# rnaarla/advanced-rag-milvus

Measured on AMD Instinct MI355X. Metric: queries_per_sec_hybrid_retrieve, higher is better.
Workload: dtype f16

## Files before the change

advanced-rag-milvus_amd/advanced_rag/_native.py:

```python
from __future__ import annotations

import ctypes
import os
import threading
from typing import Optional, Sequence, Tuple

import numpy as np

from .staging import csr_of_queries

HR_F32, HR_F16 = 0, 1
HR_METRIC_IP, HR_METRIC_COSINE, HR_METRIC_L2 = 0, 1, 2
HR_METHOD_SEMANTIC, HR_METHOD_SPARSE, HR_METHOD_DOMAIN = 1, 2, 4
HR_MAX_TOPK = 256
HR_NORM_COSINE, HR_NORM_ATAN, HR_NORM_ATAN_DIST, HR_NORM_MINMAX, HR_NORM_MINMAX_DIST = 0, 1, 2, 3, 4
HR_MAX_FUSE_LISTS = 16
HR_FUSE_RRF, HR_FUSE_WEIGHTED = 0, 1
HR_DECAY_GAUSS, HR_DECAY_EXP, HR_DECAY_LINEAR = 0, 1, 2
HR_NORM_NONE = -1
HR_MAX_BOOST_FUNCS = 8
HR_BOOST_ACTIVE, HR_BOOST_RANDOM = 1, 2
HR_BOOST_MULTIPLY, HR_BOOST_SUM = 0, 1
HR_COL_F64 = 5
HR_MAX_DEEP_K = 16384
HR_N_PHASES = 10
PHASE_NAMES = ("prep", "dense_scan", "group_select", "refine", "topk",
               "sparse_scan", "sparse_select", "sparse_refine", "sparse_topk", "finish_fused")
HR_DEBUG_FINISH_MODE, HR_DEBUG_FAIL_NEXT_BUILD, HR_DEBUG_DENSE_KERNELS, HR_DEBUG_SPARSE_RPB, HR_DEBUG_GROUP_ROWS = 1, 2, 3, 4, 5
HR_DEBUG_NO_TRIM = 6
HR_DEBUG_NO_RANGE_CLAMP = 7

_HERE = os.path.dirname(os.path.abspath(__file__))
LIB_PATH = os.path.join(os.path.dirname(_HERE), "lib", "libhbmrag.so")

_lib = None
_lib_lock = threading.Lock()


class HbmRagError(RuntimeError):

    def __init__(self, status: int, message: str):
        super().__init__(f"libhbmrag status {status}: {message}")
        self.status = status


_c = ctypes
_SIGNATURES = {
    "hr_version": (_c.c_int, []),
    "hr_create": (_c.c_int, [_c.c_int, _c.c_int64, _c.c_int, _c.c_int, _c.c_int64, _c.POINTER(_c.c_void_p)]),
    "hr_destroy": (None, [_c.c_void_p]),
    "hr_last_error": (_c.c_char_p, [_c.c_void_p]),
    "hr_set_row_offset": (_c.c_int, [_c.c_void_p, _c.c_int64]),
    "hr_reserve": (_c.c_int, [_c.c_void_p, _c.c_int64]),
    "hr_add_dense": (_c.c_int, [_c.c_void_p, _c.c_void_p, _c.c_int64]),
    "hr_add_dense_raw": (_c.c_int, [_c.c_void_p, _c.c_void_p, _c.c_int64]),
    "hr_add_dense_raw_dev": (_c.c_int, [_c.c_void_p, _c.c_void_p, _c.c_int64, _c.c_void_p]),
    "hr_add_sparse": (_c.c_int, [_c.c_void_p, _c.c_void_p, _c.c_void_p, _c.c_void_p, _c.c_int64]),
    "hr_finalize": (_c.c_int, [_c.c_void_p]),
    "hr_compact": (_c.c_int, [_c.c_void_p, _c.c_void_p, _c.c_int, _c.POINTER(_c.c_int64), _c.POINTER(_c.c_int64)]),
    "hr_save": (_c.c_int, [_c.c_void_p, _c.c_char_p]),
    "hr_load": (_c.c_int, [_c.c_char_p, _c.c_int, _c.POINTER(_c.c_void_p)]),
    "hr_get_info": (_c.c_int, [_c.c_void_p, _c.POINTER(_c.c_int64), _c.POINTER(_c.c_int32), _c.POINTER(_c.c_int32),
                               _c.POINTER(_c.c_int64)]),
    "hr_num_rows": (_c.c_int64, [_c.c_void_p]),
    "hr_num_sparse_rows": (_c.c_int64, [_c.c_void_p]),
    "hr_device_bytes": (_c.c_int64, [_c.c_void_p]),
    "hr_dense_scan_bytes": (_c.c_int64, [_c.c_void_p]),
    "hr_search_dense": (_c.c_int, [_c.c_void_p, _c.c_void_p, _c.c_int, _c.c_int, _c.c_void_p, _c.c_void_p,
                                   _c.c_void_p]),
    "hr_search_dense_range": (_c.c_int, [_c.c_void_p, _c.c_void_p, _c.c_int, _c.c_int, _c.c_void_p, _c.c_int, _c.c_void_p,
                                         _c.c_void_p, _c.c_void_p, _c.c_void_p]),
    "hr_search_sparse": (_c.c_int, [_c.c_void_p, _c.c_void_p, _c.c_void_p, _c.c_void_p, _c.c_int, _c.c_int,
                                    _c.c_float, _c.c_void_p, _c.c_void_p, _c.c_void_p]),
    "hr_search_dense_dmask": (_c.c_int, [_c.c_void_p, _c.c_void_p, _c.c_int, _c.c_int, _c.c_void_p, _c.c_void_p,
                                         _c.c_void_p]),
    "hr_search_sparse_dmask": (_c.c_int, [_c.c_void_p, _c.c_void_p, _c.c_void_p, _c.c_void_p, _c.c_int, _c.c_int,
                                          _c.c_float, _c.c_void_p, _c.c_void_p, _c.c_void_p]),
    "hr_filter_eval_expr_dev": (_c.c_int, [_c.c_void_p, _c.c_int, _c.c_void_p, _c.c_int, _c.c_int64, _c.c_void_p, _c.c_void_p,
                                           _c.c_void_p, _c.c_void_p, _c.c_void_p]),
    "hr_filter_eval_dev": (_c.c_int, [_c.c_void_p, _c.c_int, _c.c_int64, _c.c_void_p, _c.c_void_p, _c.c_void_p,
                                      _c.c_void_p, _c.c_void_p]),
    "hr_bm25_encode_dev": (_c.c_int, [_c.c_void_p, _c.c_void_p, _c.c_int, _c.c_int, _c.c_double, _c.c_double, _c.c_double, _c.c_int,
                                      _c.c_void_p, _c.c_void_p, _c.c_void_p, _c.c_void_p, _c.c_void_p]),
    "hr_hash_tokenize_dev": (_c.c_int, [_c.c_void_p, _c.c_void_p, _c.c_int, _c.c_int, _c.c_int, _c.c_void_p, _c.c_void_p, _c.c_void_p,
                                        _c.c_void_p]),
    "hr_fuse_rrf": (_c.c_int, [_c.c_void_p, _c.c_void_p, _c.c_int, _c.c_void_p, _c.c_int, _c.c_void_p, _c.c_int,
                               _c.c_double, _c.c_double, _c.c_double, _c.c_int, _c.c_void_p, _c.c_void_p,
                               _c.c_void_p, _c.c_void_p]),
    "hr_fuse_scores": (_c.c_int, [_c.c_void_p] + [_c.c_void_p, _c.c_void_p, _c.c_int, _c.c_int] * 3 +
                       [_c.c_double, _c.c_double, _c.c_double, _c.c_void_p, _c.c_void_p, _c.c_void_p, _c.c_void_p]),
    "hr_fuse_scores_dev": (_c.c_int, [_c.c_void_p, _c.c_void_p, _c.c_int, _c.c_int] * 3 +
                           [_c.c_int, _c.c_double, _c.c_double, _c.c_double, _c.c_void_p, _c.c_int, _c.c_void_p,
                            _c.c_void_p, _c.c_void_p, _c.c_void_p, _c.c_void_p]),
    "hr_fuse_lists_dev": (_c.c_int, [_c.c_void_p, _c.c_void_p, _c.c_int, _c.c_int, _c.c_int, _c.c_int, _c.c_int, _c.c_void_p,
                                     _c.c_void_p, _c.c_void_p, _c.c_int, _c.c_void_p, _c.c_void_p, _c.c_void_p, _c.c_void_p,
                                     _c.c_void_p]),
    "hr_search_dense_dev": (_c.c_int, [_c.c_void_p, _c.c_void_p, _c.c_int, _c.c_int, _c.c_void_p, _c.c_void_p,
                                       _c.c_void_p, _c.c_void_p, _c.c_void_p]),
    "hr_search_dense_range_dev": (_c.c_int, [_c.c_void_p, _c.c_void_p, _c.c_int, _c.c_int, _c.c_void_p, _c.c_void_p,
                                             _c.c_void_p, _c.c_void_p, _c.c_void_p, _c.c_void_p, _c.c_void_p]),
    "hr_search_sparse_dev": (_c.c_int, [_c.c_void_p, _c.c_void_p, _c.c_void_p, _c.c_void_p, _c.c_int, _c.c_int64,
                                        _c.c_int, _c.c_int, _c.c_void_p, _c.c_void_p, _c.c_void_p, _c.c_void_p,
                                        _c.c_void_p]),
    "hr_search_hybrid_dev": (_c.c_int, [_c.c_void_p, _c.c_void_p, _c.c_void_p, _c.c_void_p, _c.c_void_p, _c.c_int,
                                        _c.c_int64, _c.c_int, _c.c_int, _c.c_void_p, _c.c_void_p, _c.c_void_p,
                                        _c.c_void_p, _c.c_void_p]),
    "hr_hybrid_prep_dev": (_c.c_int, [_c.c_void_p, _c.c_void_p, _c.c_void_p, _c.c_void_p, _c.c_void_p, _c.c_int,
                                      _c.c_int64, _c.c_int, _c.c_int, _c.c_int, _c.c_void_p]),
    "hr_hybrid_scan_dev": (_c.c_int, [_c.c_void_p, _c.c_void_p, _c.c_void_p, _c.c_void_p, _c.c_void_p, _c.c_int,
                                      _c.c_int64, _c.c_int, _c.c_int, _c.c_void_p, _c.c_int, _c.c_void_p]),
    "hr_hybrid_finish_dev": (_c.c_int, [_c.c_void_p, _c.c_void_p, _c.c_void_p, _c.c_void_p, _c.c_void_p, _c.c_int,
                                        _c.c_int, _c.c_int, _c.c_void_p, _c.c_int, _c.c_void_p, _c.c_void_p,
                                        _c.c_void_p, _c.c_void_p]),
    "hr_fuse_rrf_dev": (_c.c_int, [_c.c_void_p, _c.c_int, _c.c_void_p, _c.c_int, _c.c_void_p, _c.c_int, _c.c_int,
                                   _c.c_double, _c.c_double, _c.c_double, _c.c_int, _c.c_int, _c.c_void_p,
                                   _c.c_void_p, _c.c_void_p, _c.c_void_p, _c.c_void_p]),
    "hr_merge_topk_dev": (_c.c_int, [_c.c_void_p, _c.c_void_p, _c.c_int, _c.c_int64, _c.c_int64, _c.c_int, _c.c_int,
                                     _c.c_int, _c.c_void_p, _c.c_void_p, _c.c_void_p]),
    "hr_merge_topk_asc_dev": (_c.c_int, [_c.c_void_p, _c.c_void_p, _c.c_int, _c.c_int64, _c.c_int64, _c.c_int, _c.c_int,
                                     _c.c_int, _c.c_void_p, _c.c_void_p, _c.c_void_p]),
    "hr_post_lists_dev": (_c.c_int, [_c.c_void_p, _c.c_int, _c.c_void_p]),
    "hr_stream_create": (_c.c_int, [_c.c_int, _c.c_int, _c.c_void_p, _c.c_int, _c.POINTER(_c.c_void_p)]),
    "hr_stream_destroy": (_c.c_int, [_c.c_int, _c.c_void_p]),
    "hr_set_scan_cus": (_c.c_int, [_c.c_void_p, _c.c_int]),
    "hr_debug_option": (_c.c_int, [_c.c_void_p, _c.c_int, _c.c_int]),
    "hr_rerank_linear_dev": (_c.c_int, [_c.c_void_p, _c.c_void_p, _c.c_void_p, _c.c_void_p, _c.c_void_p, _c.c_int,
                                        _c.c_int, _c.c_double, _c.c_double, _c.c_double, _c.c_int, _c.c_void_p,
                                        _c.c_void_p, _c.c_void_p, _c.c_void_p]),
    "hr_mmr_select_dev": (_c.c_int, [_c.c_void_p, _c.c_void_p, _c.c_void_p, _c.c_int, _c.c_int, _c.c_void_p, _c.c_void_p,
                                     _c.c_int64, _c.c_int64, _c.c_void_p, _c.c_int, _c.c_void_p, _c.c_void_p, _c.c_void_p]),
    "hr_mmr_vec_scratch_bytes": (_c.c_size_t, [_c.c_void_p, _c.c_int, _c.c_int]),
    "hr_mmr_select_vec_dev": (_c.c_int, [_c.c_void_p, _c.c_void_p, _c.c_void_p, _c.c_int, _c.c_int, _c.c_void_p, _c.c_int, _c.c_int,
                                         _c.c_void_p, _c.c_int, _c.c_void_p, _c.c_void_p, _c.c_void_p, _c.c_void_p, _c.c_void_p]),
    "hr_group_select_dev": (_c.c_int, [_c.c_void_p, _c.c_void_p, _c.c_int, _c.c_int, _c.c_void_p, _c.c_int64, _c.c_int64, _c.c_int,
                                       _c.c_void_p, _c.c_void_p, _c.c_void_p, _c.c_void_p, _c.c_void_p]),
    "hr_boost_rerank_dev": (_c.c_int, [_c.c_void_p, _c.c_void_p, _c.c_int, _c.c_void_p, _c.c_int, _c.c_int, _c.c_void_p, _c.c_int,
                                       _c.c_int64, _c.c_int, _c.c_int, _c.c_int, _c.c_int, _c.c_int, _c.c_void_p, _c.c_void_p,
                                       _c.c_void_p, _c.c_void_p, _c.c_void_p, _c.c_void_p]),
    "hr_decay_rerank_dev": (_c.c_int, [_c.c_void_p, _c.c_void_p, _c.c_int, _c.c_void_p, _c.c_int, _c.c_int, _c.c_void_p, _c.c_int,
                                       _c.c_int64, _c.c_int64, _c.c_void_p, _c.c_int, _c.c_int, _c.c_void_p, _c.c_void_p, _c.c_void_p,
                                       _c.c_void_p, _c.c_void_p]),
    "hr_mask_drop_groups_dev": (_c.c_int, [_c.c_void_p, _c.c_void_p, _c.c_int64, _c.c_void_p, _c.c_void_p, _c.c_int, _c.c_void_p]),
    "hr_group_select_n_dev": (_c.c_int, [_c.c_void_p, _c.c_void_p, _c.c_int, _c.c_int, _c.c_void_p, _c.c_int64, _c.c_int64, _c.c_int,
                                         _c.c_int, _c.c_void_p, _c.c_void_p, _c.c_void_p, _c.c_void_p, _c.c_void_p, _c.c_void_p]),
    "hr_mask_keep_groups_dev": (_c.c_int, [_c.c_void_p, _c.c_void_p, _c.c_int64, _c.c_void_p, _c.c_void_p, _c.c_int, _c.c_void_p]),
    "hr_add_layernorm_f16_dev": (_c.c_int, [_c.c_void_p, _c.c_void_p, _c.c_void_p, _c.c_void_p, _c.c_void_p, _c.c_int64,
                                            _c.c_int, _c.c_float, _c.c_void_p]),
    "hr_embed_layernorm_f16_dev": (_c.c_int, [_c.c_void_p, _c.c_void_p, _c.c_void_p, _c.c_void_p, _c.c_void_p, _c.c_void_p,
                                              _c.c_void_p, _c.c_void_p, _c.c_int64, _c.c_int, _c.c_int, _c.c_float, _c.c_int64,
                                              _c.c_int64, _c.c_void_p]),
    "hr_attention_f16_dev": (_c.c_int, [_c.c_void_p, _c.c_void_p, _c.c_void_p, _c.c_int64, _c.c_int, _c.c_int, _c.c_int,
                                        _c.c_float, _c.c_void_p]),
    "hr_attention_rows_f16_dev": (_c.c_int, [_c.c_void_p, _c.c_int64, _c.c_int64, _c.c_void_p, _c.c_void_p, _c.c_int64, _c.c_int64,
                                             _c.c_void_p, _c.c_void_p, _c.c_int64, _c.c_int, _c.c_int, _c.c_int, _c.c_int, _c.c_float,
                                             _c.c_void_p]),
    "hr_linear_rows_f16_dev": (_c.c_int, [_c.c_void_p, _c.c_int, _c.c_void_p, _c.c_void_p, _c.c_void_p, _c.c_int64, _c.c_int, _c.c_int,
                                          _c.c_int64, _c.c_void_p]),
    "hr_attention_fr_f16_dev": (_c.c_int, [_c.c_void_p, _c.c_void_p, _c.c_void_p, _c.c_int64, _c.c_int, _c.c_int, _c.c_int,
                                           _c.c_float, _c.c_void_p]),
    "hr_encoder_tail_f16_dev": (_c.c_int, [_c.c_void_p, _c.c_void_p, _c.c_int, _c.c_void_p, _c.c_int, _c.c_void_p, _c.c_void_p,
                                           _c.c_int64, _c.c_int, _c.c_int, _c.c_float, _c.c_int, _c.c_void_p]),
    "hr_mask_rows_scratch_bytes": (_c.c_size_t, [_c.c_int64]),
    "hr_mask_rows_dev": (_c.c_int, [_c.c_void_p, _c.c_int64, _c.c_int64, _c.c_int64, _c.c_int64, _c.c_void_p, _c.c_void_p,
                                    _c.c_void_p, _c.c_void_p]),
    "hr_get_dense_rows_dev": (_c.c_int, [_c.c_void_p, _c.c_void_p, _c.c_int64, _c.c_int, _c.c_void_p, _c.c_int64, _c.c_void_p,
                                         _c.c_void_p]),
    "hr_get_dense_rows": (_c.c_int, [_c.c_void_p, _c.c_void_p, _c.c_int64, _c.c_void_p]),
    "hr_get_sparse_rows_scratch_bytes": (_c.c_size_t, [_c.c_int64]),
    "hr_get_sparse_rows_dev": (_c.c_int, [_c.c_void_p, _c.c_void_p, _c.c_int64, _c.c_void_p, _c.c_void_p, _c.c_void_p, _c.c_int64,
                                          _c.c_void_p, _c.c_void_p, _c.c_void_p]),
    "hr_get_sparse_rows": (_c.c_int, [_c.c_void_p, _c.c_void_p, _c.c_int64, _c.c_void_p, _c.c_void_p, _c.c_void_p, _c.c_int64,
                                      _c.c_void_p]),
    "hr_search_dense_deep": (_c.c_int, [_c.c_void_p, _c.c_void_p, _c.c_int, _c.c_int, _c.c_int, _c.c_void_p, _c.c_int, _c.c_void_p,
                                        _c.c_void_p]),
    "hr_search_sparse_deep": (_c.c_int, [_c.c_void_p, _c.c_void_p, _c.c_void_p, _c.c_void_p, _c.c_int, _c.c_int, _c.c_int,
                                         _c.c_float, _c.c_void_p, _c.c_int, _c.c_void_p, _c.c_void_p]),
    "hr_deep_topk_scratch_bytes": (_c.c_size_t, [_c.c_int64, _c.c_int, _c.c_int]),
    "hr_deep_topk_dev": (_c.c_int, [_c.c_void_p, _c.c_void_p, _c.c_int64, _c.c_int, _c.c_int, _c.c_int, _c.c_int, _c.c_int64,
                                    _c.c_void_p, _c.c_void_p, _c.c_void_p, _c.c_void_p]),
    "hr_search_dense_deep_after": (_c.c_int, [_c.c_void_p, _c.c_void_p, _c.c_int, _c.c_int, _c.c_void_p, _c.c_void_p, _c.c_void_p,
                                              _c.c_void_p, _c.c_void_p, _c.c_void_p, _c.c_int, _c.c_void_p, _c.c_void_p]),
    "hr_search_sparse_deep_after": (_c.c_int, [_c.c_void_p, _c.c_void_p, _c.c_void_p, _c.c_void_p, _c.c_int, _c.c_int, _c.c_void_p,
                                               _c.c_void_p, _c.c_void_p, _c.c_float, _c.c_void_p, _c.c_int, _c.c_void_p,
                                               _c.c_void_p]),
    "hr_deep_topk_window_dev": (_c.c_int, [_c.c_void_p, _c.c_void_p, _c.c_int64, _c.c_int, _c.c_int, _c.c_int, _c.c_int64,
                                           _c.c_void_p, _c.c_void_p, _c.c_void_p, _c.c_void_p, _c.c_void_p]),
    "hr_set_profiling": (_c.c_int, [_c.c_void_p, _c.c_int]),
    "hr_last_kernel_ms": (_c.c_int, [_c.c_void_p, _c.c_void_p, _c.c_int]),
    "hr_last_compact_ms": (_c.c_int, [_c.c_void_p, _c.c_void_p, _c.c_int]),
}
EXPORTED_SYMBOLS = tuple(_SIGNATURES)


def load_library(path: Optional[str] = None) -> ctypes.CDLL:
    global _lib
    with _lib_lock:
        if _lib is not None and path is None:
            return _lib
        p = path or os.environ.get("HBMRAG_LIB", LIB_PATH)
        if not os.path.exists(p):
            raise FileNotFoundError(
                f"{p} not found: build it with `make -C advanced-rag-milvus_amd` "
                "(or __graft_entry__.build()); there is no CPU fallback")
        try:
            import torch
        except Exception:
            pass
        L = ctypes.CDLL(p)
        for name, (restype, argtypes) in _SIGNATURES.items():
            fn = getattr(L, name)
            fn.restype = restype
            fn.argtypes = argtypes
        if path is None:
            _lib = L
        return L


def _vp(a) -> Optional[ctypes.c_void_p]:
    if a is None:
        return None
    if isinstance(a, np.ndarray):
        return a.ctypes.data_as(ctypes.c_void_p)
    return ctypes.c_void_p(int(a))


class ShardHandle:

    def __init__(self, dim: int, dtype: int = HR_F16, metric: int = HR_METRIC_COSINE, sparse_dim: int = 0,
                 device: int = 0, _adopt: Optional[int] = None):
        self._lib = load_library()
        self._h = ctypes.c_void_p()
        if _adopt is not None:
            self._h = ctypes.c_void_p(_adopt)
            self.dim, self.dtype, self.metric, self.sparse_dim, self.device = dim, dtype, metric, sparse_dim, device
            return
        self.dim, self.dtype, self.metric, self.sparse_dim, self.device = dim, dtype, metric, sparse_dim, device
        rc = self._lib.hr_create(device, dim, dtype, metric, sparse_dim, ctypes.byref(self._h))
        if rc != 0:
            msg = (self._lib.hr_last_error(None) or b"").decode()
            self._h = ctypes.c_void_p()
            self._raise(rc, msg)

    def _raise(self, rc: int, msg: Optional[str] = None):
        if msg is None:
            msg = (self._lib.hr_last_error(self._h) or b"").decode()
        if rc == 1:
            raise ValueError(msg)
        raise HbmRagError(rc, msg)

    def _check(self, rc: int):
        if rc != 0:
            self._raise(rc)

    def close(self):
        if getattr(self, "_h", None) is not None and self._h.value:
            self._lib.hr_destroy(self._h)
            self._h = ctypes.c_void_p()

    def __del__(self):
        try:
            self.close()
        except Exception:
            pass

    def save(self, path: str):
        self._check(self._lib.hr_save(self._h, os.fsencode(path)))

    @classmethod
    def load(cls, path: str, dim: int, dtype: int = HR_F16, metric: int = HR_METRIC_COSINE, sparse_dim: int = 0,
             device: int = 0) -> "ShardHandle":
        lib = load_library()
        h = ctypes.c_void_p()
# ... 260 lines not shown
        os_ = np.empty(cap, dtype=np.float64)
        om = np.empty(cap, dtype=np.int32)
        n = ctypes.c_int32(0)
        self._check(self._lib.hr_fuse_rrf(self._h, _vp(a) if len(a) else None, len(a), _vp(b) if len(b) else None,
                                          len(b), _vp(c) if len(c) else None, len(c), wa, wb, wc, rrf_k, _vp(oi),
                                          _vp(os_), _vp(om), ctypes.byref(n)))
        return oi[:n.value].copy(), os_[:n.value].copy(), om[:n.value].copy()

    def fuse_scores(self, lists, norms, weights=(0.7, 0.3, 0.2)):
        lists = list(lists) + [((), ())] * (3 - len(lists))
        norms = list(norms) + [HR_NORM_COSINE] * (3 - len(norms))
        w = list(weights) + [0.0] * (3 - len(weights))
        ids = [np.ascontiguousarray(l[0], dtype=np.int64) for l in lists]
        sc = [np.ascontiguousarray(l[1], dtype=np.float32) for l in lists]
        if any(len(i) != len(s) for i, s in zip(ids, sc)):
            raise ValueError("a list's ids and scores differ in length")
        cap = max(sum(len(i) for i in ids), 1)
        oi = np.empty(cap, dtype=np.int64)
        os_ = np.empty(cap, dtype=np.float64)
        om = np.empty(cap, dtype=np.int32)
        n = ctypes.c_int32(0)
        args = []
        for i, s, code in zip(ids, sc, norms):
            args += [_vp(i) if len(i) else None, _vp(s) if len(i) else None, len(i), int(code)]
        self._check(self._lib.hr_fuse_scores(self._h, *args, float(w[0]), float(w[1]), float(w[2]), _vp(oi), _vp(os_),
                                             _vp(om), ctypes.byref(n)))
        return oi[:n.value].copy(), os_[:n.value].copy(), om[:n.value].copy()

    def search_dense_dev(self, d_q: int, B: int, k: int, d_ids: int, d_scores: int, d_flags: int = 0,
                         d_rowmask: int = 0, stream: int = 0):
        self._check(self._lib.hr_search_dense_dev(self._h, _vp(d_q), B, k, _vp(d_rowmask) if d_rowmask else None,
                                                  _vp(d_ids), _vp(d_scores), _vp(d_flags) if d_flags else None,
                                                  _vp(stream) if stream else None))

    def search_dense_range_dev(self, d_q: int, B: int, k: int, d_radius: int, d_range_filter: int, d_ids: int,
                               d_scores: int, d_flags: int = 0, d_rowmask: int = 0, stream: int = 0):
        self._check(self._lib.hr_search_dense_range_dev(
            self._h, _vp(d_q), B, k, _vp(d_rowmask) if d_rowmask else None, _vp(d_radius) if d_radius else None,
            _vp(d_range_filter) if d_range_filter else None, _vp(d_ids), _vp(d_scores),
            _vp(d_flags) if d_flags else None, _vp(stream) if stream else None))

    def search_sparse_dev(self, d_indptr: int, d_idx: int, d_val: int, B: int, nnz_total: int, max_q_nnz: int, k: int,
                          d_ids: int, d_scores: int, d_flags: int = 0, d_rowmask: int = 0, stream: int = 0):
        self._check(self._lib.hr_search_sparse_dev(self._h, _vp(d_indptr), _vp(d_idx), _vp(d_val), B, nnz_total,
                                                   max_q_nnz, k, _vp(d_rowmask) if d_rowmask else None, _vp(d_ids),
                                                   _vp(d_scores), _vp(d_flags) if d_flags else None,
                                                   _vp(stream) if stream else None))

    def search_hybrid_dev(self, d_q: int, d_indptr: int, d_idx: int, d_val: int, B: int, nnz_total: int,
                          max_q_nnz: int, k: int, d_ids: int, d_scores: int, d_flags: int = 0, d_rowmask: int = 0,
                          stream: int = 0):
        self._check(self._lib.hr_search_hybrid_dev(self._h, _vp(d_q), _vp(d_indptr), _vp(d_idx) if d_idx else None,
                                                   _vp(d_val) if d_val else None, B, nnz_total, max_q_nnz, k,
                                                   _vp(d_rowmask) if d_rowmask else None, _vp(d_ids), _vp(d_scores),
                                                   _vp(d_flags) if d_flags else None, _vp(stream) if stream else None))

    def hybrid_prep_dev(self, d_q: int, d_indptr: int, d_idx: int, d_val: int, B: int, nnz_total: int, max_q_nnz: int,
                        k: int, slot: int, stream: int = 0):
        self._check(self._lib.hr_hybrid_prep_dev(self._h, _vp(d_q), _vp(d_indptr), _vp(d_idx) if d_idx else None,
                                                 _vp(d_val) if d_val else None, B, nnz_total, max_q_nnz, k, slot,
                                                 _vp(stream) if stream else None))

    def hybrid_scan_dev(self, d_q: int, d_indptr: int, d_idx: int, d_val: int, B: int, nnz_total: int, max_q_nnz: int,
                        k: int, slot: int, stream: int = 0, d_rowmask: int = 0):
        self._check(self._lib.hr_hybrid_scan_dev(self._h, _vp(d_q), _vp(d_indptr), _vp(d_idx) if d_idx else None,
                                                 _vp(d_val) if d_val else None, B, nnz_total, max_q_nnz, k,
                                                 _vp(d_rowmask) if d_rowmask else None, slot,
                                                 _vp(stream) if stream else None))

    def hybrid_finish_dev(self, d_q: int, d_indptr: int, d_idx: int, d_val: int, B: int, max_q_nnz: int, k: int,
                          slot: int, d_ids: int, d_scores: int, d_flags: int = 0, stream: int = 0, d_rowmask: int = 0):
        self._check(self._lib.hr_hybrid_finish_dev(self._h, _vp(d_q), _vp(d_indptr), _vp(d_idx) if d_idx else None,
                                                   _vp(d_val) if d_val else None, B, max_q_nnz, k,
                                                   _vp(d_rowmask) if d_rowmask else None, slot, _vp(d_ids),
                                                   _vp(d_scores), _vp(d_flags) if d_flags else None,
                                                   _vp(stream) if stream else None))

    def set_scan_cus(self, n_cus: int):
        self._check(self._lib.hr_set_scan_cus(self._h, int(n_cus)))

    def debug_option(self, key: int, value: int):
        self._check(self._lib.hr_debug_option(self._h, key, value))

    def set_profiling(self, level: int):
        self._check(self._lib.hr_set_profiling(self._h, level))

    def kernel_ms(self):
        buf = np.zeros(2 * HR_N_PHASES, dtype=np.float32)
        self._check(self._lib.hr_last_kernel_ms(self._h, _vp(buf), buf.shape[0]))
        return {PHASE_NAMES[p]: (float(buf[p]), int(buf[HR_N_PHASES + p])) for p in range(HR_N_PHASES)}

    def compact_ms(self):
        buf = np.zeros(3, dtype=np.float32)
        self._check(self._lib.hr_last_compact_ms(self._h, _vp(buf), 3))
        return {"tile_gather": float(buf[0]), "call": float(buf[1]), "posting_rebuild": float(buf[2])}


def fuse_rrf_dev(d_a: int, ka: int, d_b: int, kb: int, d_c: int, kc: int, B: int, wa: float, wb: float, wc: float,
                 rrf_k: int, top_k: int, d_out_ids: int, d_out_scores: int, d_out_methods: int, d_n_out: int,
                 stream: int = 0):
    L = load_library()
    rc = L.hr_fuse_rrf_dev(_vp(d_a) if ka else None, ka, _vp(d_b) if kb else None, kb, _vp(d_c) if kc else None, kc,
                           B, wa, wb, wc, rrf_k, top_k, _vp(d_out_ids), _vp(d_out_scores), _vp(d_out_methods),
                           _vp(d_n_out), _vp(stream) if stream else None)
    if rc != 0:
        msg = (L.hr_last_error(None) or b"").decode()
        if rc == 1:
            raise ValueError(msg)
        raise HbmRagError(rc, msg)


def _raise_global(L, rc: int):
    msg = (L.hr_last_error(None) or b"").decode()
    if rc == 1:
        raise ValueError(msg)
    raise HbmRagError(rc, msg)


def fuse_scores_dev(d_a: int, d_sa: int, ka: int, norm_a: int, d_b: int, d_sb: int, kb: int, norm_b: int, d_c: int,
                    d_sc: int, kc: int, norm_c: int, B: int, wa: float, wb: float, wc: float, d_w_query: int, top_k: int,
                    d_out_ids: int, d_out_scores: int, d_out_methods: int, d_n_out: int, stream: int = 0):
    L = load_library()
    p = lambda v: _vp(v) if v else None
    rc = L.hr_fuse_scores_dev(p(d_a), p(d_sa), ka, norm_a, p(d_b), p(d_sb), kb, norm_b, p(d_c), p(d_sc), kc, norm_c, B,
                              wa, wb, wc, p(d_w_query), top_k, p(d_out_ids), p(d_out_scores), p(d_out_methods),
                              p(d_n_out), p(stream))
    if rc != 0:
        _raise_global(L, rc)


def fuse_lists_dev(d_ids: int, d_scores: int, n_lists: int, k_in: int, B: int, mode: int, rrf_k: int, norms, weights,
                   d_w_query: int, top_k: int, d_out_ids: int, d_out_scores: int, d_out_lists: int, d_n_out: int,
                   stream: int = 0):
    L = load_library()
    p = lambda v: _vp(v) if v else None
    h_norms = None if norms is None else np.ascontiguousarray(norms, dtype=np.int32)
    h_w = None if weights is None else np.ascontiguousarray(weights, dtype=np.float64)
    for name, arr in (("norms", h_norms), ("weights", h_w)):
        if arr is not None and arr.shape != (max(int(n_lists), 0),):
            raise ValueError(f"{name} must hold one value per list ({n_lists}), got shape {arr.shape}")
    rc = L.hr_fuse_lists_dev(p(d_ids), p(d_scores), n_lists, k_in, B, mode, rrf_k, _vp(h_norms), _vp(h_w), p(d_w_query),
                             top_k, p(d_out_ids), p(d_out_scores), p(d_out_lists), p(d_n_out), p(stream))
    if rc != 0:
        _raise_global(L, rc)


def mmr_select_dev(d_ids: int, d_scores: int, d_n: int, B: int, k_in: int, d_tok_indptr: int, d_tok: int, tok_rows: int,
                   first_row: int, d_lambda: int, k_out: int, d_out_pos: int, d_out_n: int, stream: int = 0):
    L = load_library()
    rc = L.hr_mmr_select_dev(_vp(d_ids) if d_ids else None, _vp(d_scores) if d_scores else None, _vp(d_n) if d_n else None,
                             B, k_in, _vp(d_tok_indptr) if d_tok_indptr else None, _vp(d_tok) if d_tok else None,
                             tok_rows, first_row, _vp(d_lambda) if d_lambda else None, k_out,
                             _vp(d_out_pos) if d_out_pos else None, _vp(d_out_n) if d_out_n else None,
                             _vp(stream) if stream else None)
    if rc != 0:
        _raise_global(L, rc)


def group_select_dev(d_ids: int, d_n: int, B: int, k_in: int, d_keys: int, key_rows: int, first_row: int, k_out: int,
                     d_out_pos: int, d_out_keys: int, d_out_n: int, d_flags: int, stream: int = 0):
    L = load_library()
    p = lambda x: _vp(x) if x else None
    rc = L.hr_group_select_dev(p(d_ids), p(d_n), B, k_in, p(d_keys), key_rows, first_row, k_out, p(d_out_pos), p(d_out_keys),
                               p(d_out_n), p(d_flags), p(stream))
    if rc != 0:
        _raise_global(L, rc)
# ... 308 lines not shown
```

advanced-rag-milvus_amd/csrc/finish.h:

```cpp
#pragma once
#include "common.h"
#include "dense.h"
#include "select.h"
#include "sparse.h"

namespace hbmrag {

constexpr int kFinishThreads = 512;
constexpr int kFinishMaxSlots = 4096;
constexpr int kFinishMaxCand = 256;
constexpr int kFinishMaxBuckets = 12288;

struct FinishMod {
    int kind;
    int group_rows;
    GroupSelArgs sel;
    TopkArgs topk;
    const uint8_t* rowmask;
    const chunk_t* tiles;
    int KT, dim, metric, dtype;
    const float* q;
    const double* qn2;
    const double* norm2;
    const double* range_bounds;
    const int64_t* indptr;
    const int32_t* idx;
    const float* val;
    const int64_t* q_indptr;
    const int32_t* q_idx;
    const float* q_val;
    int q_cap;
    int64_t n_rows;
};
struct FinishPair {
    FinishMod m[2];
    int n;
    int key_slots;
};

__host__ __device__ inline bool finish_sparse_hashed(int q_cap) { return q_cap <= kHashMaxTerms; }
inline size_t finish_lds_bytes(const FinishPair& p) {
    size_t region_b = 0;
    for (int i = 0; i < p.n; ++i) {
        const FinishMod& m = p.m[i];
        if (m.sel.two_level) region_b = region_b > (size_t)m.sel.n_buckets * 4 ? region_b : (size_t)m.sel.n_buckets * 4;
        if (m.kind == 1) {
            const size_t s = (size_t)kFilterBits / 8 +
                             (finish_sparse_hashed(m.q_cap) ? (size_t)sparse_hash_slots(m.q_cap) * 8 : (size_t)m.q_cap * 8);
            region_b = region_b > s ? region_b : s;
        } else {
            const size_t s = (size_t)m.dim * 4;
            region_b = region_b > s ? region_b : s;
        }
    }
    return (size_t)p.key_slots * 8 + region_b;
}

constexpr int kFinishBucketsPerWave = 32;
__device__ inline void bucket_max_block(const GroupSelArgs& a, int q, float* s_bmax) {
    const int lane = threadIdx.x & 63;
    const int wid = __builtin_amdgcn_readfirstlane((int)(threadIdx.x >> 6)), nw = blockDim.x >> 6;
    const float* gm = a.gmax + (int64_t)q * a.n_groups;
    for (int64_t b0 = (int64_t)wid * kFinishBucketsPerWave; b0 < a.n_buckets; b0 += (int64_t)nw * kFinishBucketsPerWave) {
        float v[kFinishBucketsPerWave];
#pragma unroll
        for (int i = 0; i < kFinishBucketsPerWave; ++i) {
            const int64_t g = (b0 + i) * kBucketGroups + lane;
            v[i] = g < a.n_groups ? gm[g] : -__builtin_inff();
        }
        float mine = -__builtin_inff();
#pragma unroll
        for (int i = 0; i < kFinishBucketsPerWave; ++i) {
            const float m = wave_max_dpp(v[i]);
            if (lane == i) mine = m;
        }
        if (lane < kFinishBucketsPerWave && b0 + lane < a.n_buckets) s_bmax[b0 + lane] = mine;
    }
}

#ifdef HR_STAMP
__device__ unsigned long long hr_finish_stamps[2][8];
#define FINISH_STAMP(i)                                                                      \
    do {                                                                                     \
        if (blockIdx.x == 0 && threadIdx.x == 0) hr_finish_stamps[blockIdx.y][i] = __builtin_amdgcn_s_memtime(); \
    } while (0)
#else
#define FINISH_STAMP(i) do {} while (0)
#endif

__global__ __launch_bounds__(kFinishThreads) void finish_kernel(FinishPair p) {
    extern __shared__ uint64_t finish_lds[];
    __shared__ SelectScratch sh;
    __shared__ int32_t sel_bucket[HR_MAX_TOPK * 2];
    __shared__ uint64_t sel[HR_MAX_TOPK];
    __shared__ int32_t s_cand[kFinishMaxCand];
    const FinishMod& a = p.m[blockIdx.y];
    const int q = blockIdx.x, tid = threadIdx.x;
    const int n_slots = a.sel.C * a.group_rows;
    uint64_t* s_key = finish_lds;
    float* s_bmax = reinterpret_cast<float*>(finish_lds + p.key_slots);

    FINISH_STAMP(0);
    if (a.sel.two_level) bucket_max_block(a.sel, q, s_bmax);
    __syncthreads();
    FINISH_STAMP(1);
    select_groups_block(a.sel, q, s_bmax, s_cand, sh, sel_bucket);
    __syncthreads();
    const int n_live_slots = min(sh.n_live, a.sel.C) * a.group_rows;
    for (int slot = n_live_slots + tid; slot < n_slots; slot += kFinishThreads) s_key[slot] = 0ull;
    FINISH_STAMP(2);
#ifdef HR_STAMP
    if (blockIdx.x == 0 && tid == 0) {
        hr_finish_stamps[blockIdx.y][5] = (unsigned long long)n_live_slots;
        hr_finish_stamps[blockIdx.y][6] = 0ull;
    }
#endif

    if (a.kind == 0) {
        float* qq = s_bmax;
        for (int k = tid; k < a.dim; k += kFinishThreads) qq[k] = a.q[(int64_t)q * a.dim + k];
        __syncthreads();
        const double qn2 = a.qn2[q];
        const double* rq = a.range_bounds ? a.range_bounds + 2 * q : nullptr;
        for (int slot = tid; slot < n_live_slots; slot += kFinishThreads) {
#ifdef HR_STAMP
            if (blockIdx.x == 0) atomicAdd(&hr_finish_stamps[blockIdx.y][6], 1ull);
#endif
            float sc = 0.f;
            int32_t row = -1;
            bool ok;
            if (a.metric == HR_METRIC_L2)
                ok = a.dtype == HR_F16
                         ? refine_dense_slot<_Float16, true>(a.tiles, a.KT, a.dim, qq, qn2, a.norm2, a.rowmask, s_cand,
                                                             a.group_rows, a.n_rows, a.metric, slot, &sc, &row)
                         : refine_dense_slot<float, true>(a.tiles, a.KT, a.dim, qq, qn2, a.norm2, a.rowmask, s_cand,
                                                          a.group_rows, a.n_rows, a.metric, slot, &sc, &row);
            else
                ok = a.dtype == HR_F16
                         ? refine_dense_slot<_Float16>(a.tiles, a.KT, a.dim, qq, qn2, a.norm2, a.rowmask, s_cand,
                                                       a.group_rows, a.n_rows, a.metric, slot, &sc, &row)
                         : refine_dense_slot<float>(a.tiles, a.KT, a.dim, qq, qn2, a.norm2, a.rowmask, s_cand,
                                                    a.group_rows, a.n_rows, a.metric, slot, &sc, &row);
            if (ok && rq) ok = a.metric == HR_METRIC_L2 ? dense_score_in_range<true>(sc, rq) : dense_score_in_range<false>(sc, rq);
            s_key[slot] = ok ? rank_key(sc, (uint32_t)row) : 0ull;
        }
    } else {
        constexpr int NW = kFinishThreads / 64;
        const int n_chains = NW * ((n_live_slots + NW * 64 - 1) / (NW * 64));
        const int chain_len = (n_live_slots + n_chains - 1) / n_chains;
        const int wid = __builtin_amdgcn_readfirstlane(tid >> 6);
        auto emit = [&](int slot, bool keep, float score, int64_t doc) { s_key[slot] = keep ? rank_key(score, (uint32_t)doc) : 0ull; };
        if (finish_sparse_hashed(a.q_cap)) {
            const int hs = sparse_hash_slots(a.q_cap);
            unsigned int* s_filter = reinterpret_cast<unsigned int*>(s_bmax);
            int32_t* s_hkey = reinterpret_cast<int32_t*>(s_filter + kFilterBits / 32);
            float* s_hval = reinterpret_cast<float*>(s_hkey + hs);
            refine_sparse_stage_query_hash(a.q_indptr, a.q_idx, a.q_val, q, a.q_cap, hs, s_filter, s_hkey, s_hval);
            for (int chain = wid; chain < n_chains; chain += NW) {
                const int slot0 = chain * chain_len;
                const int n_here = min(chain_len, n_live_slots - slot0);
                if (n_here > 0)
                    refine_sparse_chain(a.indptr, a.idx, a.val, a.rowmask, s_cand, a.group_rows, a.n_rows, slot0, n_here,
                                        SparseLookupHash{s_filter, s_hkey, s_hval, hs}, emit);
            }
        } else {
            unsigned int* s_filter = reinterpret_cast<unsigned int*>(s_bmax);
            int32_t* s_idx = reinterpret_cast<int32_t*>(s_filter + kFilterBits / 32);
            float* s_val = reinterpret_cast<float*>(s_idx + a.q_cap);
            const int nt = refine_sparse_stage_query(a.q_indptr, a.q_idx, a.q_val, q, a.q_cap, s_filter, s_idx, s_val);
            for (int chain = wid; chain < n_chains; chain += NW) {
                const int slot0 = chain * chain_len;
                const int n_here = min(chain_len, n_live_slots - slot0);
                if (n_here > 0)
                    refine_sparse_chain(a.indptr, a.idx, a.val, a.rowmask, s_cand, a.group_rows, a.n_rows, slot0, n_here,
                                        SparseLookupSorted{s_filter, s_idx, s_val, nt}, emit);
            }
        }
    }
    __syncthreads();
    FINISH_STAMP(3);
    TopkArgs t = a.topk;
    t.n = n_slots;
    select_topk_block(t, q, [&](int64_t i) -> uint64_t { return s_key[i]; }, sh, sel);
    __syncthreads();
    FINISH_STAMP(4);
}

}
```

advanced-rag-milvus_amd/csrc/hbmrag.hip:

```cpp
#include "../../include/hbmrag.h"

#include <hip/hip_runtime.h>

#include <algorithm>
#include <chrono>
#include <cmath>
#include <cstdarg>
#include <cstdio>
#include <cstdlib>
#include <cstring>
#include <map>
#include <mutex>
#include <new>
#include <shared_mutex>
#include <string>
#include <type_traits>
#include <utility>
#include <vector>

#include "common.h"
#include "attention.h"
#include "boost.h"
#include "compact.h"
#include "decay.h"
#include "deep.h"
#include "encoder_layer.h"
#include "scan_plan.h"
#include "dense.h"
#include "encoder_ops.h"
#include "filter.h"
#include "finish.h"
#include "fuse.h"
#include "fuse_lists.h"
#include "group.h"
#include "mmr.h"
#include "query.h"
#include "text.h"
#include "select.h"
#include "sparse.h"

using namespace hbmrag;

namespace {

thread_local std::string g_last_error;

struct DevBuf {
    void* p = nullptr;
    size_t cap = 0;
    DevBuf() = default;
    DevBuf(const DevBuf&) = delete;
    DevBuf& operator=(const DevBuf&) = delete;
    DevBuf(DevBuf&& o) noexcept : p(o.p), cap(o.cap) { o.p = nullptr, o.cap = 0; }
    DevBuf& operator=(DevBuf&& o) noexcept {
        if (this != &o) {
            release();
            p = o.p, cap = o.cap;
            o.p = nullptr, o.cap = 0;
        }
        return *this;
    }
    ~DevBuf() { release(); }
    hipError_t alloc_exact(size_t bytes) {
        release();
        hipError_t e = hipMalloc(&p, bytes);
        if (e == hipSuccess) cap = bytes;
        else p = nullptr;
        return e;
    }
    hipError_t ensure(size_t bytes) { return bytes <= cap ? hipSuccess : alloc_exact(bytes + bytes / 8 + 256); }
    hipError_t grow(size_t bytes, size_t keep, hipStream_t s) {
        if (bytes <= cap) return hipSuccess;
        DevBuf nb;
        hipError_t e = nb.alloc_exact(bytes + bytes / 2 + 256);
        if (e == hipSuccess && p && keep) {
            e = hipMemcpyAsync(nb.p, p, keep, hipMemcpyDeviceToDevice, s);
            if (e == hipSuccess) e = hipStreamSynchronize(s);
        }
        if (e == hipSuccess) *this = std::move(nb);
        return e;
    }
    void release() {
        if (p) (void)hipFree(p);
        p = nullptr;
        cap = 0;
    }
    template <typename T> T* as() const { return reinterpret_cast<T*>(p); }
};

enum Phase { PH_PREP = 0, PH_SCAN, PH_GSEL, PH_REFINE, PH_TOPK, PH_SSCAN, PH_SGSEL, PH_SREFINE, PH_STOPK, PH_FINISH, PH_COUNT };
static_assert(PH_COUNT == HR_N_PHASES, "phase table and ABI out of step");

struct WorkspaceQueues {
    hipStream_t stream = nullptr;
    hipStream_t side = nullptr;
    hipEvent_t ev_scan = nullptr, ev_side = nullptr;
    ~WorkspaceQueues() {
        if (stream) (void)hipStreamDestroy(stream);
        if (side) (void)hipStreamDestroy(side);
        if (ev_scan) (void)hipEventDestroy(ev_scan);
        if (ev_side) (void)hipEventDestroy(ev_side);
    }
};

struct Workspace : WorkspaceQueues {
    std::mutex mu;
    int users = 0;
    struct Workspace* sparse_ws = nullptr;
    DevBuf qfrag, qn2, gmax, bmax, cand, acut, cscore, crow, flags, qscale, qeps, qfloor, pq_n, pq_idx, pq_w;
    DevBuf qcoef, dqeps;
    DevBuf rbounds, rhi, rlo;
    DevBuf d_radius, d_rfilter;
    DevBuf d_q, d_ids, d_scores, d_mask;
    DevBuf d_qptr, d_qidx, d_qval;
    DevBuf f_ids, f_sc, f_out_ids, f_out_scores, f_out_meth, f_n;
    ~Workspace() { delete sparse_ws; }
};

struct EventSpan {
    int phase;
    hipEvent_t a, b;
};

}

struct hr_index {
    int device = 0;
    int64_t dim = 0, sparse_dim = 0;
    int dtype = HR_F16, metric = HR_METRIC_COSINE;
    int KT = 0;
    int group_rows_override = 0;
    int64_t row_offset = 0;

    DevBuf tiles, scale, norm2, max_norm;
    int64_t cap_rows = 0, n_rows = 0, n_normed = 0;
    float max_row_norm = 0.f;
    DevBuf stage;
    DevBuf bad_row;
    hipStream_t ingest_stream = nullptr;

    std::vector<int64_t> pend_indptr{0};
    std::vector<int32_t> pend_idx;
    std::vector<float> pend_val;
    std::vector<int64_t> h_range_base{0};
    std::vector<unsigned> h_range_dense;
    int64_t n_sparse = 0, n_csr = 0, nnz_csr = 0, n_sparse_built = 0;
    float max_sparse_abs = 0.f;
    bool sparse_signed = false;
    DevBuf s_indptr, s_idx, s_val, rt_off, range_base, post;
    DevBuf idle_post;
    int64_t n_ranges = 0;
    int64_t n_dense_runs = 0;

    bool finalized = false;
    int profiling = 0;
    int cu_count = 256;
    int scan_cus = 0;
    int fault_inject = 0;
    float compact_ms[3] = {};
    bool slot_prepped[HR_MAX_SLOTS] = {};

    mutable std::shared_mutex rw;
    std::mutex pool_mu;
    std::vector<Workspace*> free_ws;
    std::map<void*, Workspace*> stream_ws;
    Workspace* slot_ws[HR_MAX_SLOTS][2] = {};
    std::mutex prof_mu;
    std::vector<EventSpan> spans;
    std::vector<hipEvent_t> event_pool;
    mutable std::mutex err_mu;
    mutable std::string err;

    ~hr_index() {
        for (Workspace* w : free_ws) delete w;
        for (auto& kv : stream_ws) delete kv.second;
        for (auto& pair : slot_ws)
            for (Workspace* w : pair) delete w;
        for (auto& sp : spans) { (void)hipEventDestroy(sp.a); (void)hipEventDestroy(sp.b); }
        for (hipEvent_t e : event_pool) (void)hipEventDestroy(e);
        if (ingest_stream) (void)hipStreamDestroy(ingest_stream);
    }
};

namespace {

int fail(const hr_index* h, int code, const char* fmt, ...) {
    char buf[512];
    va_list ap;
    va_start(ap, fmt);
    vsnprintf(buf, sizeof buf, fmt, ap);
    va_end(ap);
    if (h) {
        std::lock_guard<std::mutex> g(h->err_mu);
        h->err = buf;
    }
    g_last_error = buf;
    return code;
}

#define HIP_TRY(h, expr)                                                                   \
    do {                                                                                   \
        hipError_t e__ = (expr);                                                           \
        if (e__ != hipSuccess) return fail(h, HR_EHIP, "%s: %s", #expr, hipGetErrorString(e__)); \
    } while (0)

#define HR_TRY(expr)               \
    do {                           \
        int rc__ = (expr);         \
        if (rc__ != HR_OK) return rc__; \
    } while (0)

inline size_t elem_size(int dtype) { return dtype == HR_F16 ? 2 : 4; }
inline int elems_per_chunk(int dtype) { return dtype == HR_F16 ? 8 : 4; }
inline int64_t round_up(int64_t x, int64_t m) { return (x + m - 1) / m * m; }
inline size_t tile_bytes_for_rows(const hr_index* h, int64_t rows) {
    return (size_t)(rows / kRowsPerBlock) * h->KT * 1024;
}

struct DeviceGuard {
// ... 161 lines not shown
}

template <int KT, int NRB, int GW, int NW>
hipError_t launch_scan_qreg(const ScanArgs& a) {
    const hr_index* h = a.h;
    const int64_t blocks = std::max<int64_t>(1, std::min<int64_t>(a.n_super, (int64_t)scan_cus(h) * (8 / NW)));
    hipLaunchKernelGGL((dense_scan_qreg_kernel<KT, NRB, GW, NW>), dim3((unsigned)blocks), dim3(64 * NW), 0, a.s,
                       h->tiles.as<chunk_t>(), a.qfrag, h->scale.as<float>(), a.mask, a.gmax, a.nq, h->n_rows, a.n_super);
    return hipGetLastError();
}
template <int NRB>
hipError_t launch_scan_q64(const ScanArgs& a) {
    const hr_index* h = a.h;
    const int64_t blocks = std::max<int64_t>(1, std::min<int64_t>(a.n_super, (int64_t)scan_cus(h)));
    const size_t lds = (size_t)kQregStages * 24 * 1024 + 2 * kSuperRows * sizeof(float);
    static bool ready = false;
    if (!ready) {
        hipError_t e = hipFuncSetAttribute((const void*)dense_scan_q64_kernel<24, NRB>, hipFuncAttributeMaxDynamicSharedMemorySize, (int)lds);
        if (e != hipSuccess) return e;
        ready = true;
    }
    hipLaunchKernelGGL((dense_scan_q64_kernel<24, NRB>), dim3((unsigned)blocks), dim3(256), lds, a.s, h->tiles.as<chunk_t>(),
                       a.qfrag, h->scale.as<float>(), a.mask, a.gmax, a.nq, h->n_rows, a.n_super);
    return hipGetLastError();
}
template <int NRB>
hipError_t launch_scan_gemm(const ScanArgs& a) {
    const hr_index* h = a.h;
    const int64_t n_tiles = (a.n_super * kRowBlocksPerSuper + kGemmRowBlocks - 1) / kGemmRowBlocks;
    const unsigned blocks = (unsigned)std::max<int64_t>(1, std::min<int64_t>(n_tiles, scan_cus(h)));
    hipLaunchKernelGGL((dense_scan_gemm_kernel<16, NRB>), dim3(blocks), dim3(512), 0, a.s, h->tiles.as<chunk_t>(), a.qfrag,
                       h->scale.as<float>(), a.mask, a.gmax, a.nq, h->KT, h->n_rows, a.n_super);
    return hipGetLastError();
}

template <int... Vs, typename F>
hipError_t with_constant(int v, F f) {
    hipError_t e = hipErrorInvalidValue;
    (void)((v == Vs ? (e = f(std::integral_constant<int, Vs>{}), true) : false) || ...);
    return e;
}

template <typename F>
auto with_store(int dtype, F f) {
    if (dtype == HR_F16) return f(_Float16{});
    return f(float{});
}

template <typename STORE, bool L2, bool RANGE>
hipError_t launch_scan_generic(const ScanPlan& p, const ScanArgs& a) {
    return with_constant<1, 4>(p.NRB, [&](auto nrb) {
        if (p.kind == SCAN_BIGQ) return launch_scan_bigq<STORE, 8, decltype(nrb)::value, L2, RANGE>(a);
        return with_constant<1, 2, 3, 4>(
            p.G, [&](auto g) { return launch_scan_lds<STORE, decltype(g)::value, decltype(nrb)::value, L2, RANGE>(a); });
    });
}

hipError_t launch_scan(const ScanPlan& p, const ScanArgs& a) {
    switch (p.kind) {
        case SCAN_QREG: return with_constant<1, 4>(p.NRB, [&](auto nrb) { return launch_scan_qreg<24, decltype(nrb)::value, 2, 8>(a); });
        case SCAN_Q64: return with_constant<1, 4>(p.NRB, [&](auto nrb) { return launch_scan_q64<decltype(nrb)::value>(a); });
        case SCAN_GEMM: return with_constant<1, 4>(p.NRB, [&](auto nrb) { return launch_scan_gemm<decltype(nrb)::value>(a); });
        case SCAN_LDS:
        case SCAN_BIGQ:
            return with_store(a.h->dtype, [&](auto store) {
                using STORE = decltype(store);
                if (p.range) return p.l2 ? launch_scan_generic<STORE, true, true>(p, a) : launch_scan_generic<STORE, false, true>(p, a);
                return p.l2 ? launch_scan_generic<STORE, true, false>(p, a) : launch_scan_generic<STORE, false, false>(p, a);
            });
        default: return hipErrorInvalidValue;
    }
}

struct DenseRange {
    const double* d_radius;
    const double* d_range_filter;
};

int g_dense_kernels = 0;
int g_sparse_rpb = 0;
int g_no_trim = 0;
int g_group_rows = 0;
int g_no_range_clamp = 0;

inline int64_t bucket_count(int64_t n_groups) { return (n_groups + kBucketGroups - 1) / kBucketGroups; }
int launch_group_select_pair(hr_index* h, hipStream_t s, int B, const GroupSelPair& p) {
    int64_t blocks = 0;
    for (int m = 0; m < p.n; ++m)
        if (p.m[m].two_level) blocks = std::max(blocks, (p.m[m].n_buckets + 4 * kBucketsPerWave - 1) / (4 * kBucketsPerWave));
    if (blocks > 0) {
        hipLaunchKernelGGL(bucket_max_kernel, dim3((unsigned)blocks, B, p.n), dim3(256), 0, s, p);
        HIP_TRY(h, hipGetLastError());
    }
    hipLaunchKernelGGL(select_groups_kernel, dim3(B, p.n), dim3(1024), 0, s, p);
    HIP_TRY(h, hipGetLastError());
    return HR_OK;
}
int launch_topk_pair(hr_index* h, hipStream_t s, int B, const TopkPair& p) {
    hipLaunchKernelGGL(select_topk_kernel, dim3(B, p.n), dim3(1024), 0, s, p);
    HIP_TRY(h, hipGetLastError());
    return HR_OK;
}

constexpr int kMaxSelectGroups = 448;
int next_candidate_count(int C, int64_t n_groups) {
    const int64_t all = round_up(n_groups, 16);
    if (C < kMaxSelectGroups && (int64_t)C * 4 < all) return std::min(C * 4, kMaxSelectGroups);
    return (int)all;
}

int candidate_groups_for_k(int k) {
    int c = k + std::max(16, k / 2);
    return (int)round_up(c, 16);
}

float dense_l2_rt_eps(const hr_index* h) {
    const double M = (double)h->max_row_norm * 1.0001;
    return (float)std::min(std::ldexp(1.0, -22) * 1.01 * 0.5 * M * M, 3.0e38);
}
void dense_eps(const hr_index* h, float* eps_abs, int* norm_mode) {
    const double Dp = (double)h->KT * 4 * elems_per_chunk(h->dtype);
    double unit = 2.0 * Dp * std::ldexp(1.0, -24) + 1e-6;
    unit += (h->dtype == HR_F16) ? std::ldexp(1.0, -11) * 1.01
                                 : std::ldexp(1.0, -22);
    if (h->metric == HR_METRIC_COSINE) {
        *eps_abs = (float)unit;
        *norm_mode = 0;
    } else if (h->metric == HR_METRIC_L2) {
        *eps_abs = (float)((unit + std::ldexp(1.0, -24) * 1.01) * (double)h->max_row_norm * 1.0001);
        *norm_mode = 2;
    } else {
        *eps_abs = (float)(unit * (double)h->max_row_norm * 1.0001);
        *norm_mode = 1;
    }
}

struct OutLists {
    int64_t* ids;
    float* scores;
    int32_t* flags;
};
struct FinishSide {
    Workspace* ws;
    bool sparse;
    int GR;
    int64_t n_groups;
    int C;
    const uint8_t* mask;
    TopkArgs topk;
    const float* d_q;
    const double* range_bounds;
    const int64_t* q_ptr;
    const int32_t* q_idx;
    const float* q_val;
    int stride;
    int ph_select, ph_refine, ph_topk;
};

int side_common(hr_index* h, Workspace* ws, int B, int k, int C, int GR, int64_t n_groups, const uint8_t* d_mask,
                const OutLists& out, FinishSide* f) {
    HIP_TRY(h, ws->gmax.ensure((size_t)B * n_groups * sizeof(float)));
    HIP_TRY(h, ws->bmax.ensure((size_t)B * bucket_count(n_groups) * sizeof(float)));
    HIP_TRY(h, ws->cand.ensure((size_t)B * C * sizeof(int32_t)));
    HIP_TRY(h, ws->acut.ensure((size_t)B * sizeof(float)));
    HIP_TRY(h, ws->cscore.ensure((size_t)B * C * GR * sizeof(float)));
    HIP_TRY(h, ws->crow.ensure((size_t)B * C * GR * sizeof(int32_t)));
    *f = FinishSide{};
    f->ws = ws;
    f->GR = GR;
    f->n_groups = n_groups;
    f->C = C;
    f->mask = d_mask;
    TopkArgs& t = f->topk;
    t.cscore = ws->cscore.as<float>();
    t.crow = ws->crow.as<int32_t>();
    t.n = C * GR;
    t.K = k;
    t.row_offset = h->row_offset;
    t.a_cut = ws->acut.as<float>();
    t.out_ids = out.ids;
    t.out_scores = out.scores;
    t.flags = out.flags;
    return HR_OK;
}
inline int64_t dense_super_groups(const hr_index* h) { return (h->n_rows + kSuperRows - 1) / kSuperRows; }
int dense_side(hr_index* h, Workspace* ws, const float* d_q, int B, int k, int C, const uint8_t* d_mask, const OutLists& out,
               FinishSide* f, bool ranged = false) {
    const int GR = group_rows_for(h, h->n_rows);
    HR_TRY(side_common(h, ws, B, k, C, GR, dense_super_groups(h) * (kSuperRows / GR), d_mask, out, f));
    f->d_q = d_q;
    f->ph_select = PH_GSEL, f->ph_refine = PH_REFINE, f->ph_topk = PH_TOPK;
    TopkArgs& t = f->topk;
    dense_eps(h, &t.eps_abs, &t.norm_mode);
    t.cut_floor = -INFINITY;
    t.eps_abs_q = t.norm_mode == 2 ? ws->dqeps.as<float>() : nullptr;
    t.qn2 = ws->qn2.as<double>();
    if (ranged) {
        f->range_bounds = ws->rbounds.as<double>();
        t.cut_floor_q = ws->rlo.as<float>();
    }
    return HR_OK;
}
int sparse_side(hr_index* h, Workspace* ws, const int64_t* d_qptr, const int32_t* d_qidx, const float* d_qval, int B,
                int max_q_nnz, int k, int C, const uint8_t* d_mask, const OutLists& out, FinishSide* f) {
    const int GR = group_rows_for(h, h->n_sparse);
    HR_TRY(side_common(h, ws, B, k, C, GR, (h->n_sparse + GR - 1) / GR, d_mask, out, f));
    f->sparse = true;
    f->q_ptr = d_qptr;
    f->q_idx = d_qidx;
    f->q_val = d_qval;
    f->stride = (int)round_up(std::max(max_q_nnz, 1), 64);
    f->ph_select = PH_SGSEL, f->ph_refine = PH_SREFINE, f->ph_topk = PH_STOPK;
    TopkArgs& t = f->topk;
    t.cut_floor_q = ws->qfloor.as<float>();
    t.eps_abs_q = ws->qeps.as<float>();
    t.eps_rel = (float)(std::ldexp(1.0, -11) * 1.01 + std::ldexp(1.0, -22));
    return HR_OK;
}

GroupSelArgs sel_args(const FinishSide& f) {
    GroupSelArgs a{};
    a.gmax = f.ws->gmax.as<float>();
    a.bmax = f.ws->bmax.as<float>();
    a.n_groups = f.n_groups;
    a.n_buckets = bucket_count(f.n_groups);
    a.C = f.C;
    a.two_level = f.n_groups > f.C && a.n_buckets > f.C;
    a.cand = f.ws->cand.as<int32_t>();
    a.a_cut = f.ws->acut.as<float>();
    a.K_trim = g_no_trim ? 0 : f.topk.K;
    a.eps_abs = f.topk.eps_abs;
    a.eps_rel = f.topk.eps_rel;
    a.eps_abs_q = f.topk.eps_abs_q;
    return a;
}
FinishMod finish_mod(const hr_index* h, const FinishSide& f) {
    FinishMod m{};
    m.kind = f.sparse;
    m.group_rows = f.GR;
    m.sel = sel_args(f);
    m.topk = f.topk;
    m.rowmask = f.mask;
    if (f.sparse) {
        m.indptr = h->s_indptr.as<int64_t>();
        m.idx = h->s_idx.as<int32_t>();
        m.val = h->s_val.as<float>();
        m.q_indptr = f.q_ptr;
        m.q_idx = f.q_idx;
        m.q_val = f.q_val;
        m.q_cap = f.stride;
        m.n_rows = h->n_sparse;
    } else {
        m.tiles = h->tiles.as<chunk_t>();
        m.KT = h->KT;
        m.dim = (int)h->dim;
        m.metric = h->metric;
        m.dtype = h->dtype;
        m.q = f.d_q;
        m.qn2 = f.ws->qn2.as<double>();
        m.norm2 = h->norm2.as<double>();
        m.range_bounds = f.range_bounds;
        m.n_rows = h->n_rows;
    }
    return m;
}
struct RefineBufs {
    const double* qn2;
    const int32_t* cand;
    float* cscore;
    int32_t* crow;
};
int launch_refine(hr_index* h, hipStream_t s, int B, const FinishSide& f, const RefineBufs& b) {
    if (!f.sparse) {
        const bool f16 = h->dtype == HR_F16, l2 = h->metric == HR_METRIC_L2;
        auto kern = f16 ? (l2 ? refine_dense_kernel<_Float16, true> : refine_dense_kernel<_Float16, false>)
                        : (l2 ? refine_dense_kernel<float, true> : refine_dense_kernel<float, false>);
        hipLaunchKernelGGL(kern, dim3((f.C * f.GR + 63) / 64, B), dim3(64), 0, s, h->tiles.as<chunk_t>(), h->KT, (int)h->dim,
                           f.d_q, b.qn2, h->norm2.as<double>(), f.mask, b.cand, f.C, f.GR,
                           h->n_rows, h->metric, b.cscore, b.crow, f.range_bounds);
    } else {
        const int dpw = 64;
        const bool hashed = f.stride <= kHashMaxTerms;
        const size_t lds = (size_t)kFilterBits / 8 + (hashed ? (size_t)sparse_hash_slots(f.stride) * 8 : (size_t)f.stride * 8);
        hipLaunchKernelGGL(hashed ? refine_sparse_kernel<true> : refine_sparse_kernel<false>,
                           dim3((f.C * f.GR + 4 * dpw - 1) / (4 * dpw), B), dim3(256), lds, s, h->s_indptr.as<int64_t>(),
                           h->s_idx.as<int32_t>(), h->s_val.as<float>(), f.q_ptr, f.q_idx, f.q_val, f.mask,
                           b.cand, f.C, f.GR, h->n_sparse, f.stride, dpw, b.cscore, b.crow);
    }
    HIP_TRY(h, hipGetLastError());
    return HR_OK;
}
int launch_refine(hr_index* h, hipStream_t s, int B, const FinishSide& f) {
    Workspace* ws = f.ws;
    return launch_refine(h, s, B, f, {ws->qn2.as<double>(), ws->cand.as<int32_t>(), ws->cscore.as<float>(), ws->crow.as<int32_t>()});
}

enum { PHASE_SCAN = 1, PHASE_FINISH = 2, PHASE_PREP = 4, PHASE_ALL = 7 };

int g_finish_mode = 0;
bool finish_fused_ok(int B, int n_mod, const FinishSide& f) {
    if (g_finish_mode == 1) return false;
    return ((int64_t)B * n_mod >= 64 || g_finish_mode == 2) && f.C <= kFinishMaxCand && (int64_t)f.C * f.GR <= kFinishMaxSlots &&
           bucket_count(f.n_groups) <= kFinishMaxBuckets;
}
int launch_finish(hr_index* h, hipStream_t s, int B, FinishPair& p) {
    p.key_slots = 0;
    for (int i = 0; i < p.n; ++i) p.key_slots = std::max(p.key_slots, p.m[i].sel.C * p.m[i].group_rows);
    const size_t lds = finish_lds_bytes(p);
    static bool attr_set = false;
    if (!attr_set) {
        HIP_TRY(h, hipFuncSetAttribute((const void*)finish_kernel, hipFuncAttributeMaxDynamicSharedMemorySize, 96 * 1024));
        attr_set = true;
    }
    hipLaunchKernelGGL(finish_kernel, dim3(B, p.n), dim3(kFinishThreads), lds, s, p);
    HIP_TRY(h, hipGetLastError());
    return HR_OK;
}

int finish_enqueue(hr_index* h, hipStream_t s, int B, const FinishSide* f, int n) {
    bool fused = true;
    for (int i = 0; i < n; ++i) fused = fused && finish_fused_ok(B, n, f[i]);
    if (fused) {
        Span sp(h, s, PH_FINISH);
        FinishPair p{};
        p.n = n;
        for (int i = 0; i < n; ++i) p.m[i] = finish_mod(h, f[i]);
        return launch_finish(h, s, B, p);
    }
    {
        Span sp(h, s, f[0].ph_select);
        GroupSelPair p{};
        p.n = n;
        for (int i = 0; i < n; ++i) p.m[i] = sel_args(f[i]);
        HR_TRY(launch_group_select_pair(h, s, B, p));
    }
    for (int i = 0; i < n; ++i) {
        Span sp(h, s, f[i].ph_refine);
        HR_TRY(launch_refine(h, s, B, f[i]));
    }
    {
        Span sp(h, s, f[0].ph_topk);
        TopkPair p{};
        p.n = n;
        for (int i = 0; i < n; ++i) p.m[i] = f[i].topk;
        HR_TRY(launch_topk_pair(h, s, B, p));
    }
    return HR_OK;
}

int dense_search_enqueue(hr_index* h, Workspace* ws, hipStream_t s, const float* d_q, int B, int k,
                         const uint8_t* d_mask, const OutLists& out, int C, hipEvent_t scan_done = nullptr,
                         int phases = PHASE_ALL, const DenseRange* rng = nullptr) {
    const bool ranged = rng != nullptr;
    auto plan_for = [&](int nq) {
        return scan_plan(h->KT, h->dtype, h->metric, h->n_rows, h->group_rows_override, g_dense_kernels, B, nq, ranged);
    };
    const ScanPlan first = plan_for(B);
    if (first.kind == SCAN_NONE)
        return fail(h, HR_ELIMIT, "dim=%lld: the query tile does not fit LDS and the k-chunked pass is switched off",
                    (long long)h->dim);
    const bool l2 = first.l2;
    const int chunk_q = first.chunk_q, Gmax = chunk_q / 16;
    const int n_chunks = (B + chunk_q - 1) / chunk_q;
    const size_t chunk_frag = (size_t)Gmax * h->KT * kTileChunks;
    HIP_TRY(h, ws->qfrag.ensure((size_t)n_chunks * chunk_frag * sizeof(chunk_t)));
    HIP_TRY(h, ws->qn2.ensure((size_t)B * sizeof(double)));
    if (l2) {
        HIP_TRY(h, ws->qcoef.ensure((size_t)n_chunks * chunk_q * sizeof(float)));
        HIP_TRY(h, ws->dqeps.ensure((size_t)n_chunks * chunk_q * sizeof(float)));
    }
    float* const d_coef = l2 ? ws->qcoef.as<float>() : nullptr;
    float* const d_qeps = l2 ? ws->dqeps.as<float>() : nullptr;
    const float rt_eps = l2 ? dense_l2_rt_eps(h) : 0.f;
    RangePrep rp{};
    if (ranged) {
        HIP_TRY(h, ws->rbounds.ensure((size_t)B * 2 * sizeof(double)));
        HIP_TRY(h, ws->rhi.ensure((size_t)n_chunks * chunk_q * sizeof(float)));
        HIP_TRY(h, ws->rlo.ensure((size_t)n_chunks * chunk_q * sizeof(float)));
        int norm_mode;
        dense_eps(h, &rp.eps_abs, &norm_mode);
        rp.radius = rng->d_radius;
        rp.range_filter = rng->d_range_filter;
        rp.bounds = ws->rbounds.as<double>();
        rp.hi_a = ws->rhi.as<float>();
        rp.lo_a = ws->rlo.as<float>();
        rp.max_norm = h->max_row_norm;
        rp.metric = h->metric;
        rp.no_clamp = g_no_range_clamp;
    }
    FinishSide f;
    HR_TRY(dense_side(h, ws, d_q, B, k, C, d_mask, out, &f, ranged));

    if (phases & PHASE_PREP) {
        Span sp(h, s, PH_PREP);
        const int G_total = (n_chunks - 1) * Gmax + plan_for(B - (n_chunks - 1) * chunk_q).G;
        hipLaunchKernelGGL(h->dtype == HR_F16 ? prep_queries_kernel<_Float16> : prep_queries_kernel<float>, dim3(16 * G_total),
                           dim3(256), 0, s, d_q, B, (int)h->dim, h->KT, ws->qfrag.as<chunk_t>(), ws->qn2.as<double>(), d_coef,
                           d_qeps, rt_eps, rp);
        HIP_TRY(h, hipGetLastError());
    }
    for (int c0 = 0; (phases & PHASE_SCAN) && c0 < B; c0 += chunk_q) {
        const int nq = std::min(chunk_q, B - c0);
        Span sp(h, s, PH_SCAN);
        const ScanArgs a{h, s, ws->qfrag.as<chunk_t>() + (size_t)(c0 / chunk_q) * chunk_frag, d_mask,
                         ws->gmax.as<float>() + (int64_t)c0 * f.n_groups, nq, dense_super_groups(h), l2 ? d_coef + c0 : nullptr,
                         ranged ? ws->rhi.as<float>() + c0 : nullptr};
        HIP_TRY(h, launch_scan(plan_for(nq), a));
    }
    if (scan_done) HIP_TRY(h, hipEventRecord(scan_done, s));
    return (phases & PHASE_FINISH) ? finish_enqueue(h, s, B, &f, 1) : HR_OK;
}

int sparse_ranges_per_block(const hr_index* h, int B) {
    const int forced = g_sparse_rpb;
    const int64_t pairs = (int64_t)B * h->n_ranges;
    int64_t rpb = forced > 0 ? forced : std::min<int64_t>(16, pairs / (6 * 2 * (int64_t)scan_cus(h)));
    rpb = std::max<int64_t>(rpb, (h->n_ranges + 65534) / 65535);
    return (int)std::max<int64_t>(1, rpb);
}

int sparse_search_enqueue(hr_index* h, Workspace* ws, hipStream_t s, const int64_t* d_qptr, const int32_t* d_qidx,
                          const float* d_qval, int B, int max_q_nnz, int k, const uint8_t* d_mask, const OutLists& out,
                          int C, int phases = PHASE_ALL) {
    HIP_TRY(h, ws->qscale.ensure((size_t)B * sizeof(float)));
    HIP_TRY(h, ws->qeps.ensure((size_t)B * sizeof(float)));
    HIP_TRY(h, ws->qfloor.ensure((size_t)B * sizeof(float)));
    FinishSide f;
    HR_TRY(sparse_side(h, ws, d_qptr, d_qidx, d_qval, B, max_q_nnz, k, C, d_mask, out, &f));
    if (phases & PHASE_PREP) {
        HIP_TRY(h, ws->pq_n.ensure((size_t)B * 4));
        HIP_TRY(h, ws->pq_idx.ensure((size_t)B * f.stride * 4));
        HIP_TRY(h, ws->pq_w.ensure((size_t)B * f.stride * 4));
        const float max_post_w = h->max_sparse_abs > 0.f ? std::max(h->max_sparse_abs, 0x1p-24f) : 0.f;
        hipLaunchKernelGGL(sparse_query_prep_kernel, dim3(B), dim3(256), 0, s, d_qptr, d_qidx, d_qval, max_post_w,
                           (int)h->sparse_signed, f.stride, (int)h->sparse_dim, ws->qscale.as<float>(),
                           ws->qeps.as<float>(), ws->qfloor.as<float>(), ws->pq_n.as<int32_t>(),
                           ws->pq_idx.as<int32_t>(), ws->pq_w.as<float>());
        HIP_TRY(h, hipGetLastError());
    }
    if (phases & PHASE_SCAN) {
        Span sp(h, s, PH_SSCAN);
        const int rpb = sparse_ranges_per_block(h, B);
        const unsigned chunks = (unsigned)((h->n_ranges + rpb - 1) / rpb);
        hipLaunchKernelGGL(h->n_dense_runs > 0 ? sparse_scan_kernel<true> : sparse_scan_kernel<false>,
                           dim3((unsigned)B, chunks), dim3(kScanThreads), 0, s, h->rt_off.as<unsigned int>(),
                           h->sparse_dim + 1, h->range_base.as<int64_t>(), h->post.as<uint32_t>(), ws->pq_n.as<int32_t>(),
                           ws->pq_idx.as<int32_t>(), ws->pq_w.as<float>(), f.stride, ws->qscale.as<float>(), d_mask,
                           h->n_sparse, f.n_groups, f.GR, h->n_ranges, rpb, h->idle_post.as<uint32_t>(),
                           ws->gmax.as<float>());
        HIP_TRY(h, hipGetLastError());
    }
    return (phases & PHASE_FINISH) ? finish_enqueue(h, s, B, &f, 1) : HR_OK;
}

int check_search_args(hr_index* h, int B, int k, bool dense) {
    if (!h) return fail(nullptr, HR_EINVAL, "null handle");
    if (B <= 0) return fail(h, HR_EINVAL, "batch size must be positive (got %d)", B);
    if (k <= 0) return fail(h, HR_EINVAL, "k must be positive (got %d)", k);
    if (k > HR_MAX_TOPK) return fail(h, HR_ELIMIT, "k=%d exceeds HR_MAX_TOPK=%d", k, HR_MAX_TOPK);
    if (!h->finalized) return fail(h, HR_ESTATE, "search before hr_finalize");
    if (dense && h->dim == 0) return fail(h, HR_ESTATE, "handle has no dense collection");
    if (!dense && h->sparse_dim == 0) return fail(h, HR_ESTATE, "handle has no sparse collection");
    return HR_OK;
}

int fill_empty(hr_index* h, hipStream_t s, int B, int k, int64_t* d_ids, float* d_scores, int32_t* d_flags) {
    HIP_TRY(h, hipMemsetAsync(d_ids, 0xFF, (size_t)B * k * sizeof(int64_t), s));
    HIP_TRY(h, hipMemsetAsync(d_scores, 0, (size_t)B * k * sizeof(float), s));
    if (d_flags) {
        std::vector<int32_t> ones(B, 1);
        HIP_TRY(h, hipMemcpyAsync(d_flags, ones.data(), (size_t)B * sizeof(int32_t), hipMemcpyHostToDevice, s));
        HIP_TRY(h, hipStreamSynchronize(s));
    }
    return HR_OK;
}

struct PooledWs {
    hr_index* h;
    Workspace* w;
    explicit PooledWs(hr_index* h_) : h(h_), w(take_ws(h_)) {}
    ~PooledWs() {
        if (w) give_ws(h, w);
    }
};

template <typename Stage, typename Enqueue>
int search_host(hr_index* h, int B, int k, int64_t hr_index::*rows, const uint8_t* rowmask, bool mask_on_device,
                int64_t* out_ids, float* out_scores, Stage stage_queries, Enqueue enqueue) {
    std::shared_lock<std::shared_mutex> lk(h->rw);
    DeviceGuard dg(h->device);
    const int64_t n_rows = h->*rows;
    if (n_rows == 0) {
        std::fill(out_ids, out_ids + (size_t)B * k, (int64_t)-1);
        std::fill(out_scores, out_scores + (size_t)B * k, 0.f);
        return HR_OK;
    }
    PooledWs pooled(h);
    Workspace* ws = pooled.w;
    if (!ws) return fail(h, HR_ENOMEM, "workspace allocation failed");
    hipStream_t s = ws->stream;
    HR_TRY(stage_queries(ws, s));
    HIP_TRY(h, ws->d_ids.ensure((size_t)B * k * 8));
    HIP_TRY(h, ws->d_scores.ensure((size_t)B * k * 4));
    HIP_TRY(h, ws->flags.ensure((size_t)B * 4));
    const uint8_t* d_mask = mask_on_device ? rowmask : nullptr;
    if (rowmask && !mask_on_device) {
        const size_t mb = (size_t)(n_rows + 7) / 8;
        HIP_TRY(h, ws->d_mask.ensure(mb));
        HIP_TRY(h, hipMemcpyAsync(ws->d_mask.p, rowmask, mb, hipMemcpyHostToDevice, s));
        d_mask = ws->d_mask.as<uint8_t>();
    }
    const OutLists out{ws->d_ids.as<int64_t>(), ws->d_scores.as<float>(), ws->flags.as<int32_t>()};
    const int GR = group_rows_for(h, n_rows);
    const int64_t n_row_groups = (n_rows + GR - 1) / GR;
    int C = candidate_groups_for_k(k);
    std::vector<int32_t> flags(B);
    for (;;) {
        HR_TRY(enqueue(ws, s, d_mask, out, C));
        HIP_TRY(h, hipMemcpyAsync(flags.data(), ws->flags.p, (size_t)B * 4, hipMemcpyDeviceToHost, s));
        HIP_TRY(h, hipStreamSynchronize(s));
        const bool all_exact = std::all_of(flags.begin(), flags.end(), [](int32_t f) { return f != 0; });
        if (all_exact || C >= n_row_groups) break;
        C = next_candidate_count(C, n_row_groups);
    }
    HIP_TRY(h, hipMemcpyAsync(out_ids, out.ids, (size_t)B * k * 8, hipMemcpyDeviceToHost, s));
    HIP_TRY(h, hipMemcpyAsync(out_scores, out.scores, (size_t)B * k * 4, hipMemcpyDeviceToHost, s));
    HIP_TRY(h, hipStreamSynchronize(s));
    return HR_OK;
}

int64_t dense_capacity_for(int64_t cap_rows, int64_t need_rows, bool reserving) {
    const int64_t need = round_up(need_rows, kSuperRows);
    if (reserving && cap_rows == 0) return std::max<int64_t>(need, kSuperRows);
    return std::max<int64_t>({need, round_up(cap_rows + cap_rows / 2, kSuperRows), 1024});
}

int set_dense_capacity(hr_index* h, int64_t rows) {
    DevBuf tiles, scale, norm2;
    const size_t tb = tile_bytes_for_rows(h, rows);
    if (tiles.alloc_exact(tb) != hipSuccess || scale.alloc_exact((size_t)rows * 4) != hipSuccess ||
        norm2.alloc_exact((size_t)rows * 8) != hipSuccess) {
        (void)hipGetLastError();
        return fail(h, HR_ENOMEM, "cannot allocate dense shard for %lld rows (%zu bytes)", (long long)rows, tb);
    }
    hipStream_t s = h->ingest_stream;
    HIP_TRY(h, hipMemsetAsync(tiles.p, 0, tiles.cap, s));
    HIP_TRY(h, hipMemsetAsync(scale.p, 0, scale.cap, s));
    HIP_TRY(h, hipMemsetAsync(norm2.p, 0, norm2.cap, s));
    if (h->cap_rows > 0) {
        HIP_TRY(h, hipMemcpyAsync(tiles.p, h->tiles.p, tile_bytes_for_rows(h, h->cap_rows), hipMemcpyDeviceToDevice, s));
        HIP_TRY(h, hipMemcpyAsync(scale.p, h->scale.p, (size_t)h->cap_rows * 4, hipMemcpyDeviceToDevice, s));
        HIP_TRY(h, hipMemcpyAsync(norm2.p, h->norm2.p, (size_t)h->cap_rows * 8, hipMemcpyDeviceToDevice, s));
    }
    HIP_TRY(h, hipStreamSynchronize(s));
    h->tiles = std::move(tiles);
    h->scale = std::move(scale);
    h->norm2 = std::move(norm2);
    h->cap_rows = rows;
    return HR_OK;
}

int grow_dense(hr_index* h, int64_t need_rows) {
    if (need_rows <= h->cap_rows) return HR_OK;
    return set_dense_capacity(h, dense_capacity_for(h->cap_rows, need_rows, false));
}

constexpr unsigned long long kNoBadRow = ~0ull;

template <typename SRC>
int add_dense_impl(hr_index* h, const SRC* rows, int64_t n, bool src_on_device, hipStream_t user_stream) {
    if (!h) return fail(nullptr, HR_EINVAL, "null handle");
    if (h->dim == 0) return fail(h, HR_ESTATE, "handle has no dense collection");
    if (n < 0 || (n > 0 && !rows)) return fail(h, HR_EINVAL, "bad rows/n");
    if (n == 0) return HR_OK;
    std::unique_lock<std::shared_mutex> lk(h->rw);
    DeviceGuard dg(h->device);
    HR_TRY(grow_dense(h, h->n_rows + n));
    hipStream_t s = src_on_device && user_stream ? user_stream : h->ingest_stream;
    const int64_t chunk_rows = std::max<int64_t>(1, (64ll << 20) / (h->dim * (int64_t)sizeof(SRC)));
    const int kchunks = h->KT * 4;
    unsigned long long* d_bad = h->bad_row.as<unsigned long long>();
    for (int64_t r0 = 0; r0 < n; r0 += chunk_rows) {
        const int64_t m = std::min(chunk_rows, n - r0);
        const SRC* src = rows + r0 * h->dim;
        if (!src_on_device) {
            HIP_TRY(h, h->stage.ensure((size_t)m * h->dim * sizeof(SRC)));
            HIP_TRY(h, hipMemcpyAsync(h->stage.p, src, (size_t)m * h->dim * sizeof(SRC), hipMemcpyHostToDevice, s));
            src = h->stage.as<SRC>();
        }
        const int64_t threads = m * kchunks;
        const unsigned blocks = (unsigned)((threads + 255) / 256);
        with_store(h->dtype, [&](auto store) {
            using STORE = decltype(store);
            using IN = std::conditional_t<std::is_same<STORE, float>::value, float, SRC>;
            hipLaunchKernelGGL((tile_rows_kernel<STORE, IN>), dim3(blocks), dim3(256), 0, s, reinterpret_cast<const IN*>(src), m,
                               (int)h->dim, h->KT, h->n_rows + r0, h->tiles.as<chunk_t>(), r0, d_bad);
        });
        HIP_TRY(h, hipGetLastError());
        if (!src_on_device) HIP_TRY(h, hipStreamSynchronize(s));
    }
    unsigned long long bad = kNoBadRow;
    HIP_TRY(h, hipMemcpyAsync(&bad, d_bad, sizeof bad, hipMemcpyDeviceToHost, s));
    HIP_TRY(h, hipStreamSynchronize(s));
    if (bad != kNoBadRow) {
        const int64_t threads = n * kchunks;
        hipLaunchKernelGGL(zero_rows_kernel, dim3((unsigned)((threads + 255) / 256)), dim3(256), 0, s, n, h->KT,
                           h->n_rows, h->tiles.as<chunk_t>());
        HIP_TRY(h, hipGetLastError());
        HIP_TRY(h, hipMemsetAsync(d_bad, 0xFF, sizeof bad, s));
        HIP_TRY(h, hipStreamSynchronize(s));
        return fail(h, HR_EINVAL, "dense row %lld of the batch holds a value that is NaN or infinite in the shard's %s store",
                    (long long)bad, h->dtype == HR_F16 ? "fp16" : "fp32");
    }
    h->n_rows += n;
    h->finalized = false;
    return HR_OK;
}

int validate_csr(const hr_index* h, const int64_t* indptr, const int32_t* indices, const float* values, int64_t n,
                 float* batch_max, bool* batch_neg) {
    float mx = 0.f;
    bool neg = false;
    for (int64_t r = 0; r < n; ++r) {
        if (indptr[r + 1] < indptr[r]) return fail(h, HR_EINVAL, "indptr not monotone at row %lld", (long long)r);
        int32_t prev = -1;
        for (int64_t e = indptr[r]; e < indptr[r + 1]; ++e) {
            const int32_t t = indices[e];
            if (t < 0 || t >= h->sparse_dim)
                return fail(h, HR_EINVAL, "sparse index %d out of range [0,%lld) in row %lld", t, (long long)h->sparse_dim, (long long)r);
            if (t <= prev) return fail(h, HR_EINVAL, "sparse indices must be strictly ascending (row %lld)", (long long)r);
            if (!std::isfinite(values[e])) return fail(h, HR_EINVAL, "non-finite sparse value in row %lld", (long long)r);
            if (std::fabs(values[e]) > 60000.f)
                return fail(h, HR_ELIMIT, "sparse weight %g in row %lld exceeds the fp16 posting range", (double)values[e], (long long)r);
            mx = std::max(mx, std::fabs(values[e]));
            neg |= values[e] < 0.f;
            prev = t;
        }
    }
    *batch_max = mx;
    *batch_neg = neg;
    return HR_OK;
// ... 159 lines not shown
    if (span) HIP_TRY(h, hipEventRecord(span[1], s));
    hipLaunchKernelGGL(compact_row_values_kernel, dim3((unsigned)((kept + 255) / 256)), dim3(256), 0, s, h->scale.as<float>(),
                       h->norm2.as<double>(), d_src_of, kept, out->scale.as<float>(), out->norm2.as<double>(),
                       out->max_norm.as<unsigned int>());
    HIP_TRY(h, hipGetLastError());
    return HR_OK;
}

struct CompactSparse {
    DevBuf indptr, idx, val, stats;
    int64_t nnz = 0;
};
int compact_sparse(hr_index* h, hipStream_t s, const uint32_t* d_src_of, int64_t kept, CompactSparse* out) {
    if (kept == 0) return HR_OK;
    DevBuf block_off, total;
    if (out->indptr.alloc_exact((size_t)(kept + 1) * 8) != hipSuccess || out->stats.alloc_exact(8) != hipSuccess ||
        total.alloc_exact(8) != hipSuccess) {
        (void)hipGetLastError();
        return fail(h, HR_ENOMEM, "cannot allocate the compacted sparse rows (%lld) beside the old ones", (long long)kept);
    }
    const RowLength len{h->s_indptr.as<int64_t>(), d_src_of};
    HR_TRY(compact_scan_blocks(h, s, len, kept, block_off, total.as<unsigned long long>()));
    hipLaunchKernelGGL(compact_indptr_kernel, dim3((unsigned)((kept + kCompactBlock - 1) / kCompactBlock)), dim3(kCompactBlock), 0, s,
                       len, kept, block_off.as<unsigned long long>(), out->indptr.as<int64_t>());
    HIP_TRY(h, hipGetLastError());
    unsigned long long nnz = 0;
    HIP_TRY(h, hipMemcpyAsync(&nnz, total.p, 8, hipMemcpyDeviceToHost, s));
    HIP_TRY(h, hipStreamSynchronize(s));
    out->nnz = (int64_t)nnz;
    if (out->idx.alloc_exact((size_t)std::max<int64_t>(out->nnz, 1) * 4) != hipSuccess ||
        out->val.alloc_exact((size_t)std::max<int64_t>(out->nnz, 1) * 4) != hipSuccess) {
        (void)hipGetLastError();
        return fail(h, HR_ENOMEM, "cannot allocate the compacted sparse entries (%lld) beside the old ones", (long long)out->nnz);
    }
    HIP_TRY(h, hipMemsetAsync(out->stats.p, 0, 8, s));
    hipLaunchKernelGGL(compact_csr_kernel, dim3((unsigned)((kept + 3) / 4)), dim3(256), 0, s, h->s_indptr.as<int64_t>(),
                       h->s_idx.as<int32_t>(), h->s_val.as<float>(), d_src_of, kept, out->indptr.as<int64_t>(),
                       out->idx.as<int32_t>(), out->val.as<float>(), out->stats.as<unsigned int>());
    HIP_TRY(h, hipGetLastError());
    return HR_OK;
}

}

extern "C" {

int hr_version(void) { return 12000; }

const char* hr_last_error(const hr_index* h) {
    if (!h) return g_last_error.c_str();
    std::lock_guard<std::mutex> g(h->err_mu);
    g_last_error = h->err;
    return g_last_error.c_str();
}

int hr_create(int device, int64_t dim, int dtype, int metric, int64_t sparse_dim, hr_index** out) {
    if (!out) return fail(nullptr, HR_EINVAL, "out is null");
    *out = nullptr;
    if (dim < 0 || sparse_dim < 0 || (dim == 0 && sparse_dim == 0))
        return fail(nullptr, HR_EINVAL, "need dim > 0 and/or sparse_dim > 0");
    if (dim > HR_MAX_DIM) return fail(nullptr, HR_ELIMIT, "dim=%lld exceeds HR_MAX_DIM=%d", (long long)dim, HR_MAX_DIM);
    if (dtype != HR_F32 && dtype != HR_F16) return fail(nullptr, HR_EINVAL, "unknown dtype %d", dtype);
    if (metric != HR_METRIC_IP && metric != HR_METRIC_COSINE && metric != HR_METRIC_L2) return fail(nullptr, HR_EINVAL, "unknown metric %d", metric);
    if (sparse_dim > (1ll << 24)) return fail(nullptr, HR_ELIMIT, "sparse_dim too large");
    int count = 0;
    hipError_t e = hipGetDeviceCount(&count);
    if (e != hipSuccess || count <= 0) {
        (void)hipGetLastError();
        return fail(nullptr, HR_EHIP, "no HIP device available (%s); libhbmrag has no CPU fallback",
                    e == hipSuccess ? "device count 0" : hipGetErrorString(e));
    }
    if (device < 0 || device >= count) return fail(nullptr, HR_EINVAL, "device %d out of range (0..%d)", device, count - 1);
    hr_index* h = new (std::nothrow) hr_index();
    if (!h) return fail(nullptr, HR_ENOMEM, "out of host memory");
    h->device = device;
    h->dim = dim;
    h->dtype = dtype;
    h->metric = metric;
    h->sparse_dim = sparse_dim;
    if (dim > 0) {
        const int tile_elems = 4 * elems_per_chunk(dtype);
        h->KT = (int)round_up((dim + tile_elems - 1) / tile_elems, 4);
    }
    h->group_rows_override = g_group_rows;
    DeviceGuard dg(device);
    hipDeviceProp_t prop;
    if (hipGetDeviceProperties(&prop, device) == hipSuccess) h->cu_count = prop.multiProcessorCount;
    uint32_t idle[256];
    for (unsigned l = 0; l < 256; ++l) idle[l] = filler_posting(l / 4);
    if (hipStreamCreateWithFlags(&h->ingest_stream, hipStreamNonBlocking) != hipSuccess ||
        h->max_norm.alloc_exact(4) != hipSuccess || hipMemset(h->max_norm.p, 0, 4) != hipSuccess ||
        h->bad_row.alloc_exact(8) != hipSuccess || hipMemset(h->bad_row.p, 0xFF, 8) != hipSuccess ||
        h->idle_post.alloc_exact(sizeof idle) != hipSuccess ||
        hipMemcpy(h->idle_post.p, idle, sizeof idle, hipMemcpyHostToDevice) != hipSuccess) {
        int rc = fail(nullptr, HR_EHIP, "device %d initialisation failed: %s", device, hipGetErrorString(hipGetLastError()));
        delete h;
        return rc;
    }
    *out = h;
    return HR_OK;
}

void hr_destroy(hr_index* h) {
    if (!h) return;
    DeviceGuard dg(h->device);
    (void)hipDeviceSynchronize();
    delete h;
}

int hr_set_row_offset(hr_index* h, int64_t first_row) {
    if (!h) return fail(nullptr, HR_EINVAL, "null handle");
    if (first_row < 0) return fail(h, HR_EINVAL, "row offset must be >= 0");
    h->row_offset = first_row;
    return HR_OK;
}

int hr_reserve(hr_index* h, int64_t n_rows) {
    if (!h) return fail(nullptr, HR_EINVAL, "null handle");
    if (h->dim == 0) return fail(h, HR_ESTATE, "handle has no dense collection");
    if (n_rows < 0 || n_rows > (1ll << 31) - 64) return fail(h, HR_ELIMIT, "row count out of range");
    std::unique_lock<std::shared_mutex> lk(h->rw);
    DeviceGuard dg(h->device);
    if (n_rows <= h->cap_rows) return HR_OK;
    return set_dense_capacity(h, dense_capacity_for(h->cap_rows, n_rows, true));
}

int hr_add_dense(hr_index* h, const float* rows, int64_t n) {
    return add_dense_impl<float>(h, rows, n, false, nullptr);
}

int hr_add_dense_raw(hr_index* h, const void* rows, int64_t n) {
    if (!h) return fail(nullptr, HR_EINVAL, "null handle");
    if (h->dtype == HR_F16) return add_dense_impl<_Float16>(h, static_cast<const _Float16*>(rows), n, false, nullptr);
    return add_dense_impl<float>(h, static_cast<const float*>(rows), n, false, nullptr);
}

int hr_add_dense_raw_dev(hr_index* h, const void* d_rows, int64_t n, void* stream) {
    if (!h) return fail(nullptr, HR_EINVAL, "null handle");
    if (h->dtype == HR_F16)
        return add_dense_impl<_Float16>(h, static_cast<const _Float16*>(d_rows), n, true, (hipStream_t)stream);
    return add_dense_impl<float>(h, static_cast<const float*>(d_rows), n, true, (hipStream_t)stream);
}

int hr_add_sparse(hr_index* h, const int64_t* indptr, const int32_t* indices, const float* values, int64_t n) {
    if (!h) return fail(nullptr, HR_EINVAL, "null handle");
    if (h->sparse_dim == 0) return fail(h, HR_ESTATE, "handle has no sparse collection");
    if (n < 0 || (n > 0 && !indptr)) return fail(h, HR_EINVAL, "bad indptr/n");
    if (n == 0) return HR_OK;
    const int64_t nnz = indptr[n] - indptr[0];
    if (nnz < 0 || (nnz > 0 && (!indices || !values))) return fail(h, HR_EINVAL, "bad indices/values");
    float batch_max = 0.f;
    bool batch_neg = false;
    HR_TRY(validate_csr(h, indptr, indices, values, n, &batch_max, &batch_neg));
    std::unique_lock<std::shared_mutex> lk(h->rw);
    if (h->n_sparse + n > (1ll << 31) - 64) return fail(h, HR_ELIMIT, "too many sparse rows");
    try {
        const int64_t base = h->pend_indptr.back() - indptr[0];
        h->pend_indptr.reserve(h->pend_indptr.size() + n);
        for (int64_t r = 1; r <= n; ++r) h->pend_indptr.push_back(indptr[r] + base);
        h->pend_idx.insert(h->pend_idx.end(), indices + indptr[0], indices + indptr[n]);
        h->pend_val.insert(h->pend_val.end(), values + indptr[0], values + indptr[n]);
    } catch (const std::exception&) {
        return fail(h, HR_ENOMEM, "out of host memory staging sparse rows");
    }
    h->n_sparse += n;
    h->max_sparse_abs = std::max(h->max_sparse_abs, batch_max);
    h->sparse_signed = h->sparse_signed || batch_neg;
    h->finalized = false;
    return HR_OK;
}

int hr_finalize(hr_index* h) {
    if (!h) return fail(nullptr, HR_EINVAL, "null handle");
    std::unique_lock<std::shared_mutex> lk(h->rw);
    DeviceGuard dg(h->device);
    hipStream_t s = h->ingest_stream;
    if ((h->dim > 0 && h->n_normed < h->n_rows) || (h->sparse_dim > 0 && h->n_sparse_built != h->n_sparse))
        HIP_TRY(h, hipDeviceSynchronize());
    if (h->dim > 0 && h->n_normed < h->n_rows) {
        const int64_t n = h->n_rows - h->n_normed;
        const unsigned blocks = (unsigned)((n + 255) / 256);
        with_store(h->dtype, [&](auto store) {
            hipLaunchKernelGGL((row_norms_kernel<decltype(store)>), dim3(blocks), dim3(256), 0, s, h->tiles.as<chunk_t>(), h->KT,
                               h->n_normed, n, h->metric, h->norm2.as<double>(), h->scale.as<float>(),
                               h->max_norm.as<unsigned int>());
        });
        HIP_TRY(h, hipGetLastError());
        unsigned int bits = 0;
        HIP_TRY(h, hipMemcpyAsync(&bits, h->max_norm.p, 4, hipMemcpyDeviceToHost, s));
        HIP_TRY(h, hipStreamSynchronize(s));
        std::memcpy(&h->max_row_norm, &bits, 4);
        h->n_normed = h->n_rows;
    }
    if (h->sparse_dim > 0 && (h->n_sparse_built != h->n_sparse || h->n_csr != h->n_sparse)) HR_TRY(build_sparse(h));
    h->finalized = true;
    return HR_OK;
}

int hr_compact(hr_index* h, const uint8_t* keep, int on_device, int64_t* kept_dense, int64_t* kept_sparse) {
    if (!h) return fail(nullptr, HR_EINVAL, "null handle");
    if (!keep) return fail(h, HR_EINVAL, "null keep mask");
    std::unique_lock<std::shared_mutex> lk(h->rw);
    DeviceGuard dg(h->device);
    if (!h->finalized) return fail(h, HR_ESTATE, "hr_compact before hr_finalize (pending rows must be flushed first)");
    using clk = std::chrono::steady_clock;
    const clk::time_point t_call = clk::now();
    struct Events {
        hipEvent_t e[2] = {nullptr, nullptr};
        ~Events() { for (hipEvent_t x : e) if (x) (void)hipEventDestroy(x); }
    } ev;
    bool timed = false;
    if (h->profiling && (hipEventCreate(&ev.e[0]) != hipSuccess || hipEventCreate(&ev.e[1]) != hipSuccess))
        return fail(h, HR_EHIP, "cannot create the profiling events");
    HIP_TRY(h, hipDeviceSynchronize());
    hipStream_t s = h->ingest_stream;
    const bool dense = h->dim > 0 && h->n_rows > 0, sparse = h->sparse_dim > 0 && h->n_sparse > 0;
    const int64_t n = std::max(h->n_rows, h->n_sparse);
    if (kept_dense) *kept_dense = h->n_rows;
    if (kept_sparse) *kept_sparse = h->n_sparse;
    if (n == 0) return HR_OK;

    DevBuf mask_buf;
    const unsigned long long* d_mask = reinterpret_cast<const unsigned long long*>(keep);
    if (!on_device) {
        const size_t words = (size_t)((n + 63) / 64);
        if (mask_buf.alloc_exact(words * 8) != hipSuccess) {
            (void)hipGetLastError();
            return fail(h, HR_ENOMEM, "cannot allocate the keep mask");
        }
        HIP_TRY(h, hipMemsetAsync(mask_buf.p, 0, words * 8, s));
        HIP_TRY(h, hipMemcpyAsync(mask_buf.p, keep, (size_t)((n + 7) / 8), hipMemcpyHostToDevice, s));
        d_mask = mask_buf.as<unsigned long long>();
    }
    DevBuf map_d, map_s;
    int64_t kd = 0, ks = 0;
    if (dense) HR_TRY(compact_row_map(h, s, d_mask, h->n_rows, map_d, &kd));
    if (sparse) {
        if (dense && h->n_sparse == h->n_rows) ks = kd;
        else HR_TRY(compact_row_map(h, s, d_mask, h->n_sparse, map_s, &ks));
    }
    if (kd == h->n_rows && ks == h->n_sparse) return HR_OK;
    const uint32_t* src_d = map_d.as<uint32_t>();
    const uint32_t* src_s = map_s.p ? map_s.as<uint32_t>() : src_d;
    CompactDense nd;
    CompactSparse nsp;
    if (dense && kd < h->n_rows) {
        timed = h->profiling && kd > 0;
        HR_TRY(compact_dense(h, s, src_d, kd, &nd, timed ? ev.e : nullptr));
    }
    if (sparse && ks < h->n_sparse) HR_TRY(compact_sparse(h, s, src_s, ks, &nsp));
    unsigned int norm_bits = 0, stats[2] = {0u, 0u};
    if (nd.max_norm.p) HIP_TRY(h, hipMemcpyAsync(&norm_bits, nd.max_norm.p, 4, hipMemcpyDeviceToHost, s));
    if (nsp.stats.p) HIP_TRY(h, hipMemcpyAsync(stats, nsp.stats.p, 8, hipMemcpyDeviceToHost, s));
    HIP_TRY(h, hipStreamSynchronize(s));

    auto wall_ms = [](clk::time_point a) { return std::chrono::duration<float, std::milli>(clk::now() - a).count(); };
    h->compact_ms[0] = h->compact_ms[2] = 0.f;
    if (timed) (void)hipEventElapsedTime(&h->compact_ms[0], ev.e[0], ev.e[1]);

    if (dense && kd < h->n_rows) {
        h->tiles = std::move(nd.tiles);
        h->scale = std::move(nd.scale);
        h->norm2 = std::move(nd.norm2);
        h->max_norm = std::move(nd.max_norm);
        h->cap_rows = nd.cap_rows;
        h->n_rows = h->n_normed = kd;
        std::memcpy(&h->max_row_norm, &norm_bits, 4);
    }
    if (kept_dense) *kept_dense = h->n_rows;
    if (sparse && ks < h->n_sparse) {
        h->s_indptr = std::move(nsp.indptr);
        h->s_idx = std::move(nsp.idx);
        h->s_val = std::move(nsp.val);
        h->n_sparse = h->n_csr = ks;
        h->nnz_csr = nsp.nnz;
        std::memcpy(&h->max_sparse_abs, &stats[0], 4);
        h->sparse_signed = stats[1] != 0;
        h->rt_off.release();
        h->range_base.release();
        h->post.release();
        std::vector<int64_t>{0}.swap(h->h_range_base);
        std::vector<unsigned>().swap(h->h_range_dense);
        h->n_sparse_built = 0;
        h->n_ranges = 0;
        h->n_dense_runs = 0;
        h->finalized = false;
        if (kept_sparse) *kept_sparse = ks;
        const clk::time_point t_build = clk::now();
        HR_TRY(build_sparse(h));
        h->compact_ms[2] = wall_ms(t_build);
        h->finalized = true;
    }
    h->compact_ms[1] = wall_ms(t_call);
    return HR_OK;
}

namespace {
struct SnapHeader {
    char magic[8];
    int32_t version, dtype, metric, KT;
    int64_t dim, sparse_dim, n_rows, cap_rows, n_sparse, nnz, row_offset;
    float max_row_norm, max_sparse_abs;
    int64_t file_bytes;
};
const char kSnapMagic[8] = {'H', 'B', 'M', 'R', 'A', 'G', '0', '2'};

struct File {
    FILE* f = nullptr;
    ~File() { if (f) fclose(f); }
};

int stream_out(hr_index* h, FILE* f, const void* dptr, size_t bytes) {
    std::vector<char> buf(std::min<size_t>(bytes, 64u << 20));
    for (size_t off = 0; off < bytes; off += buf.size()) {
        const size_t n = std::min(buf.size(), bytes - off);
        HIP_TRY(h, hipMemcpy(buf.data(), (const char*)dptr + off, n, hipMemcpyDeviceToHost));
        if (fwrite(buf.data(), 1, n, f) != n) return fail(h, HR_EINVAL, "snapshot write failed");
    }
    return HR_OK;
}
int stream_in(hr_index* h, FILE* f, void* dptr, size_t bytes) {
    std::vector<char> buf(std::min<size_t>(bytes, 64u << 20));
    for (size_t off = 0; off < bytes; off += buf.size()) {
        const size_t n = std::min(buf.size(), bytes - off);
        if (fread(buf.data(), 1, n, f) != n) return fail(h, HR_EINVAL, "snapshot truncated");
        HIP_TRY(h, hipMemcpy((char*)dptr + off, buf.data(), n, hipMemcpyHostToDevice));
    }
    return HR_OK;
}

struct Section {
    void* dev;
    size_t bytes;
};
struct Sections {
    Section s[6];
    int n_dense = 0, n = 0;
    Sections(const hr_index* h, const SnapHeader& hd) {
        if (hd.dim > 0 && hd.n_rows > 0) {
            s[n++] = {h->tiles.p, tile_bytes_for_rows(h, hd.cap_rows)};
            s[n++] = {h->scale.p, (size_t)hd.cap_rows * 4};
            s[n++] = {h->norm2.p, (size_t)hd.cap_rows * 8};
        }
        n_dense = n;
        if (hd.n_sparse > 0) {
            s[n++] = {h->s_indptr.p, (size_t)(hd.n_sparse + 1) * 8};
            s[n++] = {h->s_idx.p, (size_t)hd.nnz * 4};
            s[n++] = {h->s_val.p, (size_t)hd.nnz * 4};
        }
    }
    int64_t bytes() const {
        int64_t t = 0;
        for (int i = 0; i < n; ++i) t += (int64_t)s[i].bytes;
        return t;
    }
};

int save_to(hr_index* h, FILE* f) {
    SnapHeader hd{};
    std::memcpy(hd.magic, kSnapMagic, 8);
    hd.version = 2; hd.dtype = h->dtype; hd.metric = h->metric; hd.KT = h->KT;
    hd.dim = h->dim; hd.sparse_dim = h->sparse_dim; hd.n_rows = h->n_rows;
    hd.cap_rows = h->dim ? round_up(std::max<int64_t>(h->n_rows, 1), kSuperRows) : 0;
    hd.n_sparse = h->n_sparse; hd.nnz = h->nnz_csr; hd.row_offset = h->row_offset;
    hd.max_row_norm = h->max_row_norm; hd.max_sparse_abs = h->max_sparse_abs;
    const Sections body(h, hd);
    hd.file_bytes = (int64_t)sizeof hd + body.bytes();
    if (fwrite(&hd, sizeof hd, 1, f) != 1) return fail(h, HR_EINVAL, "snapshot write failed");
    for (int i = 0; i < body.n; ++i) HR_TRY(stream_out(h, f, body.s[i].dev, body.s[i].bytes));
    return HR_OK;
}

int forward_error(const hr_index* h, int rc, const char* prefix = "") {
    return fail(nullptr, rc, "%s%s", prefix, hr_last_error(h));
}
}

// ... 32 lines not shown
    SnapHeader hd{};
    if (fread(&hd, sizeof hd, 1, file.f) != 1 || std::memcmp(hd.magic, kSnapMagic, 8) != 0 || hd.version != 2)
        return fail(nullptr, HR_EINVAL, "%s is not a libhbmrag snapshot (version 2)", path);
    if (hd.n_rows < 0 || hd.n_sparse < 0 || hd.nnz < 0 || hd.cap_rows < hd.n_rows || hd.n_sparse > (1ll << 31) - 64 ||
        hd.nnz > (1ll << 40) || !(hd.max_sparse_abs >= 0.f) || !(hd.max_row_norm >= 0.f) ||
        !std::isfinite(hd.max_row_norm))
        return fail(nullptr, HR_EINVAL, "corrupt snapshot header");
    if (fseek(file.f, 0, SEEK_END) != 0 || (int64_t)ftell(file.f) != hd.file_bytes || fseek(file.f, (long)sizeof hd, SEEK_SET) != 0)
        return fail(nullptr, HR_EINVAL, "snapshot truncated or padded: %s does not hold the %lld bytes its header announces", path,
                    (long long)hd.file_bytes);
    hr_index* h = nullptr;
    HR_TRY(hr_create(device, hd.dim, hd.dtype, hd.metric, hd.sparse_dim, &h));
    struct Guard { hr_index* h; bool keep = false; ~Guard() { if (!keep) hr_destroy(h); } } guard{h};
    if (h->KT != hd.KT) return fail(nullptr, HR_EINVAL, "snapshot tile layout (KT=%d) differs from this build (KT=%d)", hd.KT, h->KT);
    h->row_offset = hd.row_offset;
    DeviceGuard dg(device);
    const bool dense = hd.dim > 0 && hd.n_rows > 0;
    if (dense) {
        if (hd.cap_rows != round_up(hd.n_rows, kSuperRows)) return fail(nullptr, HR_EINVAL, "corrupt snapshot header (row capacity)");
        HR_TRY(hr_reserve(h, hd.cap_rows));
    }
    const Sections body(h, hd);
    for (int i = 0; i < body.n_dense; ++i) {
        const int rc = stream_in(h, file.f, body.s[i].dev, body.s[i].bytes);
        if (rc != HR_OK) return forward_error(h, rc);
    }
    if (dense) {
        h->n_rows = h->n_normed = hd.n_rows;
        h->max_row_norm = hd.max_row_norm;
        unsigned int bits;
        std::memcpy(&bits, &hd.max_row_norm, 4);
        if (hipMemcpy(h->max_norm.p, &bits, 4, hipMemcpyHostToDevice) != hipSuccess)
            return fail(nullptr, HR_EHIP, "snapshot upload failed");
    }
    if (hd.n_sparse > 0) {
        if (hd.sparse_dim <= 0) return fail(nullptr, HR_EINVAL, "corrupt snapshot header (sparse rows without a sparse collection)");
        const Section* sp = body.s + body.n_dense;
        std::vector<int64_t> ptr(sp[0].bytes / 8);
        std::vector<int32_t> idx(sp[1].bytes / 4);
        std::vector<float> val(sp[2].bytes / 4);
        const bool ok = fread(ptr.data(), 1, sp[0].bytes, file.f) == sp[0].bytes &&
                        fread(idx.data(), 1, sp[1].bytes, file.f) == sp[1].bytes &&
                        fread(val.data(), 1, sp[2].bytes, file.f) == sp[2].bytes;
        if (!ok || ptr.front() != 0 || ptr.back() != hd.nnz)
            return fail(nullptr, HR_EINVAL, "snapshot truncated or corrupt (sparse section)");
        for (int64_t r = 0; r < hd.n_sparse; ++r)
            if (ptr[r + 1] < ptr[r] || ptr[r + 1] > hd.nnz) return fail(nullptr, HR_EINVAL, "snapshot corrupt (sparse row pointers)");
        const int rc = hr_add_sparse(h, ptr.data(), idx.data(), val.data(), hd.n_sparse);
        if (rc != HR_OK) return forward_error(h, rc, "snapshot corrupt (sparse section): ");
    }
    const int rc = hr_finalize(h);
    if (rc != HR_OK) return forward_error(h, rc);
    guard.keep = true;
    *out = h;
    return HR_OK;
}

int hr_load(const char* path, int device, hr_index** out) {
    if (!path || !out) return fail(nullptr, HR_EINVAL, "null argument");
    *out = nullptr;
    try {
        return load_impl(path, device, out);
    } catch (const std::bad_alloc&) {
        return fail(nullptr, HR_ENOMEM, "out of host memory loading snapshot");
    } catch (const std::exception& e) {
        return fail(nullptr, HR_EINVAL, "snapshot refused: %s", e.what());
    }
}

int hr_get_info(const hr_index* h, int64_t* dim, int32_t* dtype, int32_t* metric, int64_t* sparse_dim) {
    if (!h) return fail(nullptr, HR_EINVAL, "null handle");
    if (dim) *dim = h->dim;
    if (dtype) *dtype = h->dtype;
    if (metric) *metric = h->metric;
    if (sparse_dim) *sparse_dim = h->sparse_dim;
    return HR_OK;
}

int64_t hr_num_rows(const hr_index* h) { return h ? h->n_rows : 0; }
int64_t hr_num_sparse_rows(const hr_index* h) { return h ? h->n_sparse : 0; }
int64_t hr_device_bytes(const hr_index* h) {
    if (!h) return 0;
    size_t t = 0;
    for (const DevBuf* b : {&h->tiles, &h->scale, &h->norm2, &h->s_indptr, &h->s_idx, &h->s_val, &h->rt_off,
                            &h->range_base, &h->post})
        t += b->cap;
    return (int64_t)t;
}
int64_t hr_dense_scan_bytes(const hr_index* h) {
    if (!h || h->dim == 0) return 0;
    const int64_t dpad = (int64_t)h->KT * 4 * elems_per_chunk(h->dtype);
    return h->n_rows * dpad * (int64_t)elem_size(h->dtype) + h->n_rows * 4;
}

static int check_query_nnz(hr_index* h, int max_q_nnz) {
    if (max_q_nnz < 0 || max_q_nnz > HR_MAX_QUERY_NNZ) return fail(h, HR_ELIMIT, "query nnz exceeds HR_MAX_QUERY_NNZ");
    return HR_OK;
}

int hr_search_dense_dev(hr_index* h, const float* d_q, int B, int k, const uint8_t* d_rowmask, int64_t* d_ids,
                        float* d_scores, int32_t* d_flags, void* stream) {
    HR_TRY(check_search_args(h, B, k, true));
    if (!d_q || !d_ids || !d_scores) return fail(h, HR_EINVAL, "null buffer");
    std::shared_lock<std::shared_mutex> lk(h->rw);
    DeviceGuard dg(h->device);
    hipStream_t s = (hipStream_t)stream;
    if (h->n_rows == 0) return fill_empty(h, s, B, k, d_ids, d_scores, d_flags);
    StreamWs ws_held;
    Workspace* ws = ws_for_stream(h, stream, ws_held);
    if (!ws) return fail(h, HR_ENOMEM, "workspace allocation failed");
    return dense_search_enqueue(h, ws, s, d_q, B, k, d_rowmask, {d_ids, d_scores, d_flags}, candidate_groups_for_k(k));
}

int hr_search_dense_range_dev(hr_index* h, const float* d_q, int B, int k, const uint8_t* d_rowmask, const double* d_radius,
                              const double* d_range_filter, int64_t* d_ids, float* d_scores, int32_t* d_flags,
                              void* stream) {
    HR_TRY(check_search_args(h, B, k, true));
    if (!d_q || !d_ids || !d_scores) return fail(h, HR_EINVAL, "null buffer");
    std::shared_lock<std::shared_mutex> lk(h->rw);
    DeviceGuard dg(h->device);
    hipStream_t s = (hipStream_t)stream;
    if (h->n_rows == 0) return fill_empty(h, s, B, k, d_ids, d_scores, d_flags);
    StreamWs ws_held;
    Workspace* ws = ws_for_stream(h, stream, ws_held);
    if (!ws) return fail(h, HR_ENOMEM, "workspace allocation failed");
    const DenseRange rng{d_radius, d_range_filter};
    return dense_search_enqueue(h, ws, s, d_q, B, k, d_rowmask, {d_ids, d_scores, d_flags}, candidate_groups_for_k(k), nullptr,
                                PHASE_ALL, &rng);
}

int hr_search_sparse_dev(hr_index* h, const int64_t* d_q_indptr, const int32_t* d_q_idx, const float* d_q_val, int B,
                         int64_t q_nnz_total, int max_q_nnz, int k, const uint8_t* d_rowmask, int64_t* d_ids,
                         float* d_scores, int32_t* d_flags, void* stream) {
    HR_TRY(check_search_args(h, B, k, false));
    if (!d_q_indptr || !d_ids || !d_scores || (q_nnz_total > 0 && (!d_q_idx || !d_q_val)))
        return fail(h, HR_EINVAL, "null buffer");
    HR_TRY(check_query_nnz(h, max_q_nnz));
    std::shared_lock<std::shared_mutex> lk(h->rw);
    DeviceGuard dg(h->device);
    hipStream_t s = (hipStream_t)stream;
    if (h->n_sparse == 0) return fill_empty(h, s, B, k, d_ids, d_scores, d_flags);
    StreamWs ws_held;
    Workspace* ws = ws_for_stream(h, stream, ws_held);
    if (!ws) return fail(h, HR_ENOMEM, "workspace allocation failed");
    return sparse_search_enqueue(h, ws, s, d_q_indptr, d_q_idx, d_q_val, B, max_q_nnz, k, d_rowmask,
                                 {d_ids, d_scores, d_flags}, candidate_groups_for_k(k));
}

static int check_hybrid_args(hr_index* h, int B, int k, bool buffers_ok) {
    HR_TRY(check_search_args(h, B, k, true));
    HR_TRY(check_search_args(h, B, k, false));
    return buffers_ok ? HR_OK : fail(h, HR_EINVAL, "null buffer");
}
static OutLists sparse_half(int B, int k, int64_t* d_ids, float* d_scores, int32_t* d_flags) {
    return {d_ids + (size_t)B * k, d_scores + (size_t)B * k, d_flags ? d_flags + B : nullptr};
}

int hr_search_hybrid_dev(hr_index* h, const float* d_q, const int64_t* d_q_indptr, const int32_t* d_q_idx,
                         const float* d_q_val, int B, int64_t q_nnz_total, int max_q_nnz, int k,
                         const uint8_t* d_rowmask, int64_t* d_ids, float* d_scores, int32_t* d_flags, void* stream) {
    HR_TRY(check_hybrid_args(h, B, k, d_q && d_q_indptr && d_ids && d_scores && (q_nnz_total <= 0 || (d_q_idx && d_q_val))));
    HR_TRY(check_query_nnz(h, max_q_nnz));
    std::shared_lock<std::shared_mutex> lk(h->rw);
    DeviceGuard dg(h->device);
    hipStream_t s = (hipStream_t)stream;
    const OutLists so = sparse_half(B, k, d_ids, d_scores, d_flags);
    StreamWs ws_held;
    Workspace* ws = ws_for_stream(h, stream, ws_held);
    if (!ws) return fail(h, HR_ENOMEM, "workspace allocation failed");
    if (!ws->side) {
        HIP_TRY(h, hipStreamCreateWithFlags(&ws->side, hipStreamNonBlocking));
        HIP_TRY(h, hipEventCreateWithFlags(&ws->ev_scan, hipEventDisableTiming));
        HIP_TRY(h, hipEventCreateWithFlags(&ws->ev_side, hipEventDisableTiming));
// ... 391 lines not shown
        if (e != hipSuccess) return fail(nullptr, HR_EHIP, "hipFuncSetAttribute: %s", hipGetErrorString(e));
        attr_set = true;
    }
    hipLaunchKernelGGL(bm25_encode_kernel, dim3((unsigned)n_docs), dim3(kBm25Threads), lds, (hipStream_t)stream, a);
    hipError_t e = hipGetLastError();
    if (e != hipSuccess) return fail(nullptr, HR_EHIP, "bm25_encode_kernel: %s", hipGetErrorString(e));
    return HR_OK;
}

int hr_hash_tokenize_dev(const uint8_t* d_text, const int64_t* d_off, int n, int max_len, int vocab, int64_t* d_ids,
                         int32_t* d_lens, int32_t* d_flags, void* stream) {
    if (n < 0 || !d_off || !d_lens || !d_flags || (n > 0 && (!d_text || !d_ids))) return fail(nullptr, HR_EINVAL, "bad tokenizer arguments");
    if (max_len < 3 || vocab <= 1000) return fail(nullptr, HR_EINVAL, "max_len must be >= 3 and the vocabulary larger than 1000");
    if (n == 0) return HR_OK;
    TokArgs a{};
    a.text = d_text; a.off = d_off; a.n = n; a.max_len = max_len; a.vocab = vocab;
    a.ids = d_ids; a.lens = d_lens; a.flags = d_flags;
    hipLaunchKernelGGL(hash_tokenize_kernel, dim3((unsigned)n), dim3(kTokThreads), 0, (hipStream_t)stream, a);
    hipError_t e = hipGetLastError();
    if (e != hipSuccess) return fail(nullptr, HR_EHIP, "hash_tokenize_kernel: %s", hipGetErrorString(e));
    return HR_OK;
}

int hr_stream_create(int device, int priority, const uint32_t* cu_mask, int n_words, void** out_stream) {
    if (!out_stream || n_words < 0 || (n_words > 0 && !cu_mask)) return fail(nullptr, HR_EINVAL, "bad stream arguments");
    *out_stream = nullptr;
    DeviceGuard dg(device);
    hipStream_t s = nullptr;
    hipError_t e;
    if (n_words > 0) {
        e = hipExtStreamCreateWithCUMask(&s, (uint32_t)n_words, cu_mask);
    } else {
        int lo = 0, hi = 0;
        (void)hipDeviceGetStreamPriorityRange(&lo, &hi);
        e = hipStreamCreateWithPriority(&s, hipStreamNonBlocking, std::max(hi, std::min(lo, priority)));
    }
    if (e != hipSuccess) {
        (void)hipGetLastError();
        return fail(nullptr, HR_EHIP, "stream creation failed: %s", hipGetErrorString(e));
    }
    *out_stream = (void*)s;
    return HR_OK;
}

int hr_stream_destroy(int device, void* stream) {
    if (!stream) return HR_OK;
    DeviceGuard dg(device);
    hipError_t e = hipStreamDestroy((hipStream_t)stream);
    if (e != hipSuccess) return fail(nullptr, HR_EHIP, "hipStreamDestroy: %s", hipGetErrorString(e));
    return HR_OK;
}

int hr_set_scan_cus(hr_index* h, int n_cus) {
    if (!h) return fail(nullptr, HR_EINVAL, "null handle");
    if (n_cus < 0) return fail(h, HR_EINVAL, "n_cus must be >= 0");
    h->scan_cus = n_cus;
    return HR_OK;
}

int hr_debug_option(hr_index* h, int key, int value) {
    switch (key) {
        case HR_DEBUG_FINISH_MODE:
            if (value < 0 || value > 2) return fail(h, HR_EINVAL, "finish mode must be 0, 1 or 2");
            g_finish_mode = value;
            return HR_OK;
        case HR_DEBUG_DENSE_KERNELS:
            if (value < 0 || value > 31) return fail(h, HR_EINVAL, "dense kernel mask must be 0..31");
            g_dense_kernels = value;
            return HR_OK;
        case HR_DEBUG_SPARSE_RPB:
            if (value < 0 || value > 64) return fail(h, HR_EINVAL, "ranges per block must be 0..64");
            g_sparse_rpb = value;
            return HR_OK;
        case HR_DEBUG_GROUP_ROWS:
            if (value != 0 && value != 16 && value != 64) return fail(h, HR_EINVAL, "group rows must be 0, 16 or 64");
            g_group_rows = value;
            return HR_OK;
        case HR_DEBUG_NO_TRIM:
            g_no_trim = value != 0;
            return HR_OK;
        case HR_DEBUG_NO_RANGE_CLAMP:
            g_no_range_clamp = value != 0;
            return HR_OK;
        case HR_DEBUG_FAIL_NEXT_BUILD:
            if (!h) return fail(nullptr, HR_EINVAL, "null handle");
            h->fault_inject = value ? 1 : 0;
            return HR_OK;
        default:
            return fail(h, HR_EINVAL, "unknown debug option %d", key);
    }
}

int hr_rerank_linear_dev(const int64_t* d_ids, const double* d_scores, const int32_t* d_methods, const int32_t* d_n,
                         const double* d_recency, int B, int k_in, double base_w, double method_bonus,
                         double recency_w, int k_out, int64_t* d_out_ids, double* d_out_scores, double* d_out_orig,
                         void* stream) {
    if (B <= 0 || k_in <= 0 || k_out <= 0) return fail(nullptr, HR_EINVAL, "bad rerank sizes");
    if (k_in > HR_MAX_TOPK) return fail(nullptr, HR_ELIMIT, "k_in exceeds HR_MAX_TOPK=%d", HR_MAX_TOPK);
    if (!d_ids || !d_scores || !d_methods || !d_n || !d_out_ids || !d_out_scores || !d_out_orig)
        return fail(nullptr, HR_EINVAL, "null buffer");
    hipLaunchKernelGGL(rerank_linear_kernel, dim3(B), dim3(256), 0, (hipStream_t)stream, d_ids, d_scores, d_methods, d_n,
                       d_recency, k_in, base_w, method_bonus, recency_w, k_out, d_out_ids, d_out_scores, d_out_orig);
    hipError_t e = hipGetLastError();
    if (e != hipSuccess) return fail(nullptr, HR_EHIP, "rerank_linear_kernel: %s", hipGetErrorString(e));
    return HR_OK;
}

int hr_mmr_select_dev(const int64_t* d_ids, const double* d_scores, const int32_t* d_n, int B, int k_in,
                      const int64_t* d_tok_indptr, const int32_t* d_tok, int64_t tok_rows, int64_t first_row,
                      const double* d_lambda, int k_out, int32_t* d_out_pos, int32_t* d_out_n, void* stream) {
    if (B <= 0 || k_in <= 0 || k_out <= 0 || k_out > k_in || tok_rows < 0) return fail(nullptr, HR_EINVAL, "bad mmr sizes");
    if (k_in > kFuseMax) return fail(nullptr, HR_ELIMIT, "k_in exceeds 3 * HR_MAX_TOPK = %d", kFuseMax);
    if (!d_ids || !d_scores || !d_n || !d_lambda || !d_out_pos || !d_out_n) return fail(nullptr, HR_EINVAL, "null buffer");
    if (tok_rows > 0 ? (!d_tok_indptr || !d_tok) : (d_tok_indptr || d_tok))
        return fail(nullptr, HR_EINVAL, "token arrays must be given exactly when tok_rows > 0");
    hipLaunchKernelGGL(mmr_select_kernel, dim3(B), dim3(256), 0, (hipStream_t)stream, d_ids, d_scores, d_n, k_in, d_tok_indptr,
                       d_tok, tok_rows, first_row, d_lambda, k_out, d_out_pos, d_out_n);
    hipError_t e = hipGetLastError();
    if (e != hipSuccess) return fail(nullptr, HR_EHIP, "mmr_select_kernel: %s", hipGetErrorString(e));
    return HR_OK;
}

int hr_group_select_dev(const int64_t* d_ids, const int32_t* d_n, int B, int k_in, const int64_t* d_keys, int64_t key_rows,
                        int64_t first_row, int k_out, int32_t* d_out_pos, int64_t* d_out_keys, int32_t* d_out_n, int32_t* d_flags,
                        void* stream) {
    if (B < 0 || k_in <= 0 || k_out <= 0 || k_out > k_in || key_rows < 0 || first_row < 0) return fail(nullptr, HR_EINVAL, "bad group sizes");
    if (k_in > kFuseMax) return fail(nullptr, HR_ELIMIT, "k_in exceeds 3 * HR_MAX_TOPK = %d", kFuseMax);
    if (B == 0) return HR_OK;
    if (!d_ids || !d_out_pos || !d_out_n) return fail(nullptr, HR_EINVAL, "null buffer");
    if (key_rows > 0 && !d_keys) return fail(nullptr, HR_EINVAL, "key_rows > 0 needs the key column");
    hipLaunchKernelGGL(group_select_kernel, dim3(B), dim3(256), 0, (hipStream_t)stream, d_ids, d_n, k_in, d_keys, key_rows, first_row,
                       k_out, d_out_pos, d_out_keys, d_out_n, d_flags);
    hipError_t e = hipGetLastError();
    if (e != hipSuccess) return fail(nullptr, HR_EHIP, "group_select_kernel: %s", hipGetErrorString(e));
    return HR_OK;
}

int hr_decay_rerank_dev(const int64_t* d_ids, const void* d_scores, int score_is_f64, const int32_t* d_n, int B, int k_in,
                        const void* d_col, int col_kind, int64_t col_rows, int64_t first_row, const hr_decay_query* d_params,
                        int norm, int k_out, int32_t* d_out_pos, int64_t* d_out_ids, double* d_out_scores, int32_t* d_out_n,
                        void* stream) {
    if (B < 0 || k_in <= 0 || k_out <= 0 || k_out > k_in || col_rows < 0 || first_row < 0) return fail(nullptr, HR_EINVAL, "bad decay sizes");
    if (k_in > kFuseMax) return fail(nullptr, HR_ELIMIT, "k_in exceeds 3 * HR_MAX_TOPK = %d", kFuseMax);
    if (norm < HR_NORM_NONE || norm > HR_NORM_MINMAX_DIST) return fail(nullptr, HR_EINVAL, "bad norm code %d", norm);
    if (col_kind != HR_COL_I64 && col_kind != HR_COL_F32 && col_kind != HR_COL_F64) return fail(nullptr, HR_EINVAL, "bad column kind %d", col_kind);
    if (B == 0) return HR_OK;
    if (!d_ids || !d_scores || !d_params || !d_out_pos || !d_out_ids || !d_out_scores || !d_out_n) return fail(nullptr, HR_EINVAL, "null buffer");
    if (col_rows > 0 && !d_col) return fail(nullptr, HR_EINVAL, "col_rows > 0 needs the column");
    hipLaunchKernelGGL(decay_rerank_kernel, dim3(B), dim3(256), 0, (hipStream_t)stream, d_ids, d_scores, score_is_f64, d_n, k_in, d_col,
                       col_kind, col_rows, first_row, d_params, norm, k_out, d_out_pos, d_out_ids, d_out_scores, d_out_n);
    hipError_t e = hipGetLastError();
    if (e != hipSuccess) return fail(nullptr, HR_EHIP, "decay_rerank_kernel: %s", hipGetErrorString(e));
    return HR_OK;
}

int hr_boost_rerank_dev(const int64_t* d_ids, const void* d_scores, int score_is_f64, const int32_t* d_n, int B, int k_in,
                        const hr_boost_func* d_funcs, int n_funcs, int64_t first_row, int function_mode, int boost_mode, int norm,
                        int ascending, int k_out, int32_t* d_out_pos, int64_t* d_out_ids, double* d_out_scores,
                        int32_t* d_out_matched, int32_t* d_out_n, void* stream) {
    if (B < 0 || k_in <= 0 || k_out <= 0 || k_out > k_in || n_funcs <= 0 || first_row < 0) return fail(nullptr, HR_EINVAL, "bad boost sizes");
    if (k_in > kFuseMax) return fail(nullptr, HR_ELIMIT, "k_in exceeds 3 * HR_MAX_TOPK = %d", kFuseMax);
    if (n_funcs > HR_MAX_BOOST_FUNCS) return fail(nullptr, HR_ELIMIT, "n_funcs exceeds HR_MAX_BOOST_FUNCS = %d", HR_MAX_BOOST_FUNCS);
    if (norm < HR_NORM_NONE || norm > HR_NORM_MINMAX_DIST) return fail(nullptr, HR_EINVAL, "bad norm code %d", norm);
    if (function_mode < HR_BOOST_MULTIPLY || function_mode > HR_BOOST_SUM || boost_mode < HR_BOOST_MULTIPLY || boost_mode > HR_BOOST_SUM)
        return fail(nullptr, HR_EINVAL, "bad boost modes %d / %d", function_mode, boost_mode);
    if (B == 0) return HR_OK;
// ... 1105 lines not shown
```

include/hbmrag.h:

```cpp
#ifndef HBMRAG_H
#define HBMRAG_H

#include <stdint.h>
#include <stddef.h>

#if defined(HR_BUILD)
#define HR_API __attribute__((visibility("default")))
#else
#define HR_API
#endif

#ifdef __cplusplus
extern "C" {
#endif

typedef struct hr_index hr_index;

typedef enum hr_status {
    HR_OK = 0,
    HR_EINVAL = 1,
    HR_ESTATE = 2,
    HR_EHIP = 3,
    HR_ENOMEM = 4,
    HR_ELIMIT = 5
// ... 202 lines not shown
    int32_t n_flag_rows;
    int32_t reserved2;
    int32_t* agg_flags;
    const double* w_query;
    int32_t fusion;
    int32_t norm[3];
} hr_post_args;
HR_API int hr_post_lists_dev(const hr_post_args* args, int B, void* stream);

enum { HR_COL_I64 = 0, HR_COL_I64_VS_F64 = 1, HR_COL_F32 = 2, HR_COL_STR16 = 3 };
enum { HR_OP_EQ = 0, HR_OP_NE = 1, HR_OP_LT = 2, HR_OP_LE = 3, HR_OP_GT = 4, HR_OP_GE = 5 };
#define HR_MAX_FILTER_TERMS 16
typedef struct hr_filter_term {
    int32_t kind;
    int32_t op;
    const void* col;
    int64_t ival;
    double dval;
    float fval;
    uint32_t reserved;
    uint64_t key[2];
} hr_filter_term;
HR_API int hr_filter_eval_dev(const hr_filter_term* terms, int n_terms, int64_t n_rows, const uint8_t* d_deleted,
                       uint8_t* d_mask, uint8_t* d_undecided, int32_t* d_counts, void* stream);

enum { HR_OP_IN = 6 };
enum { HR_COL_TOKENS = 4, HR_OP_MATCH = 7 };
enum { HR_FILTER_AND = -1, HR_FILTER_OR = -2, HR_FILTER_NOT = -3 };
#define HR_MAX_FILTER_PROGRAM 64
#define HR_MAX_FILTER_SET_BYTES 65536
typedef struct hr_filter_leaf {
    hr_filter_term term;
    const void* set;
    int32_t n_set, reserved;
} hr_filter_leaf;
HR_API int hr_filter_eval_expr_dev(const hr_filter_leaf* leaves, int n_leaves, const int32_t* program, int n_program,
                                   int64_t n_rows, const uint8_t* d_deleted, uint8_t* d_mask, uint8_t* d_undecided,
                                   int32_t* d_counts, void* stream);

HR_API size_t hr_mask_rows_scratch_bytes(int64_t n_rows);
HR_API int hr_mask_rows_dev(const uint8_t* d_mask, int64_t n_rows, int64_t first_row, int64_t offset, int64_t limit,
                     int64_t* d_rows, int64_t* d_counts, void* d_scratch, void* stream);
HR_API int hr_get_dense_rows_dev(hr_index* h, const int64_t* d_rows, int64_t n, int out_dtype, void* d_out,
                          int64_t out_stride, int32_t* d_missing, void* stream);
HR_API int hr_get_dense_rows(hr_index* h, const int64_t* rows, int64_t n, float* out);
HR_API size_t hr_get_sparse_rows_scratch_bytes(int64_t n);
HR_API int hr_get_sparse_rows_dev(hr_index* h, const int64_t* d_rows, int64_t n, int64_t* d_out_indptr, int32_t* d_out_idx,
                           float* d_out_val, int64_t cap, int64_t* d_counts, void* d_scratch, void* stream);
HR_API int hr_get_sparse_rows(hr_index* h, const int64_t* rows, int64_t n, int64_t* out_indptr, int32_t* out_idx,
                       float* out_val, int64_t cap, int64_t* nnz_total);

HR_API int hr_bm25_encode_dev(const uint8_t* d_text, const int64_t* d_off, int n_docs, int sparse_dim, double k1, double b,
                       double avgdl, int cap, int32_t* d_idx, float* d_val, int32_t* d_nnz, int32_t* d_flags, void* stream);

HR_API int hr_hash_tokenize_dev(const uint8_t* d_text, const int64_t* d_off, int n, int max_len, int vocab, int64_t* d_ids,
                         int32_t* d_lens, int32_t* d_flags, void* stream);

HR_API int hr_add_layernorm_f16_dev(const void* d_x, const void* d_residual, const void* d_gamma, const void* d_beta,
                             void* d_out, int64_t rows, int hidden, float eps, void* stream);

HR_API int hr_embed_layernorm_f16_dev(const int64_t* d_ids, const int64_t* d_types, const void* d_word, const void* d_pos,
                               const void* d_seg, const void* d_gamma, const void* d_beta, void* d_out, int64_t n_seq, int T,
                               int hidden, float eps, int64_t n_word, int64_t n_seg, void* stream);

HR_API int hr_attention_f16_dev(const void* d_qkv, const int32_t* d_lengths, void* d_out, int64_t n_seq, int T, int heads,
                         int head_dim, float scale, void* stream);
HR_API int hr_attention_rows_f16_dev(const void* d_q, int64_t q_seq_stride, int64_t q_token_stride, const void* d_k, const void* d_v,
                              int64_t kv_seq_stride, int64_t kv_token_stride, const int32_t* d_lengths, void* d_out,
                              int64_t n_seq, int T, int n_queries, int heads, int head_dim, float scale, void* stream);

HR_API int hr_linear_rows_f16_dev(const void* d_x, int x_fr, const void* d_w_packed, const float* d_bias, void* d_out, int64_t rows,
                           int K, int N, int64_t out_stride, void* stream);
HR_API int hr_attention_fr_f16_dev(const void* d_qkv, const int32_t* d_lengths, void* d_out_fr, int64_t n_seq, int T, int heads,
                            int head_dim, float scale, void* stream);
HR_API int hr_encoder_tail_f16_dev(const void* d_attn_fr, const void* d_x, int x_fr, void* d_out, int out_fr, const void* d_wstream,
                            const float* d_tables, int64_t rows, int hidden, int intermediate, float eps, int gelu_erf,
                            void* stream);

HR_API int hr_stream_create(int device, int priority, const uint32_t* cu_mask, int n_words, void** out_stream);
HR_API int hr_stream_destroy(int device, void* stream);
HR_API int hr_set_scan_cus(hr_index* h, int n_cus);

enum { HR_DEBUG_FINISH_MODE = 1, HR_DEBUG_FAIL_NEXT_BUILD = 2, HR_DEBUG_DENSE_KERNELS = 3, HR_DEBUG_SPARSE_RPB = 4,
       HR_DEBUG_GROUP_ROWS = 5, HR_DEBUG_NO_TRIM = 6, HR_DEBUG_NO_RANGE_CLAMP = 7 };
HR_API int hr_debug_option(hr_index* h, int key, int value);

#define HR_N_PHASES 10
HR_API int hr_set_profiling(hr_index* h, int enabled);
HR_API int hr_last_kernel_ms(hr_index* h, float* out_ms, int n);
HR_API int hr_last_compact_ms(hr_index* h, float* out_ms, int n);
HR_API int64_t hr_dense_scan_bytes(const hr_index* h);

#ifdef __cplusplus
}
#endif
#endif
```

Before: 34060.

## Add int8 quantized dense scan with error-bounded finish refinement

Builds an int8 copy of the f16 dense tiles with per-row scales and residual error bounds, and adds an MFMA i8 scan kernel that computes upper-bound group maxima. Queries are split into a hi/lo int8 pair so the bound stays safe. A new finish mode (kind 2) refines candidates exactly in f16 and pulls in extra groups whose bound exceeds the kth score threshold. The aim is to halve the bytes read by the memory-bound dense scan, at the cost of extra memory, a quantization pass at finalize, and a more complex finish with possible overflow.

```diff
diff --git a/advanced-rag-milvus_amd/advanced_rag/_native.py b/advanced-rag-milvus_amd/advanced_rag/_native.py
--- a/advanced-rag-milvus_amd/advanced_rag/_native.py
+++ b/advanced-rag-milvus_amd/advanced_rag/_native.py
@@ -29,6 +29,7 @@
 HR_DEBUG_FINISH_MODE, HR_DEBUG_FAIL_NEXT_BUILD, HR_DEBUG_DENSE_KERNELS, HR_DEBUG_SPARSE_RPB, HR_DEBUG_GROUP_ROWS = 1, 2, 3, 4, 5
 HR_DEBUG_NO_TRIM = 6
 HR_DEBUG_NO_RANGE_CLAMP = 7
+HR_DEBUG_I8_SCAN = 8
 
 _HERE = os.path.dirname(os.path.abspath(__file__))
 LIB_PATH = os.path.join(os.path.dirname(_HERE), "lib", "libhbmrag.so")
@@ -188,6 +189,7 @@
     "hr_set_profiling": (_c.c_int, [_c.c_void_p, _c.c_int]),
     "hr_last_kernel_ms": (_c.c_int, [_c.c_void_p, _c.c_void_p, _c.c_int]),
     "hr_last_compact_ms": (_c.c_int, [_c.c_void_p, _c.c_void_p, _c.c_int]),
+    "hr_bound_finish_stats": (_c.c_int, [_c.c_void_p, _c.c_void_p]),
 }
 EXPORTED_SYMBOLS = tuple(_SIGNATURES)
 
@@ -614,6 +616,11 @@
     def debug_option(self, key: int, value: int):
         self._check(self._lib.hr_debug_option(self._h, key, value))
 
+    def bound_finish_stats(self) -> dict:
+        buf = np.zeros(4, dtype=np.uint64)
+        self._check(self._lib.hr_bound_finish_stats(self._h, _vp(buf)))
+        return {"queries": int(buf[0]), "extra_groups": int(buf[1]), "max_extra_groups": int(buf[2]), "overflowed": int(buf[3])}
+
     def set_profiling(self, level: int):
         self._check(self._lib.hr_set_profiling(self._h, level))
 
diff --git a/advanced-rag-milvus_amd/csrc/dense_i8.h b/advanced-rag-milvus_amd/csrc/dense_i8.h
--- /dev/null
+++ b/advanced-rag-milvus_amd/csrc/dense_i8.h
@@ -0,0 +1,272 @@
+#pragma once
+#include "common.h"
+#include "dense.h"
+
+namespace hbmrag {
+
+typedef int i32x4_t __attribute__((ext_vector_type(4)));
+
+__host__ __device__ inline int i8_tiles_per_row(int64_t dim) { return (int)(((dim + 63) / 64 + 3) / 4 * 4); }
+__host__ __device__ inline float i8_err_gain(int KT8) { return 1.0001f + sqrtf((float)(KT8 * 64)) / 64000.f; }
+
+__global__ void quantize_rows_kernel(const chunk_t* __restrict__ tiles, int KT, int KT8, int dim, int64_t row0, int64_t n,
+                                     int metric, const double* __restrict__ norm2, chunk_t* __restrict__ tiles8,
+                                     float* __restrict__ scale8, float* __restrict__ err8) {
+    const int64_t r = row0 + (int64_t)blockIdx.x * blockDim.x + threadIdx.x;
+    if (r >= row0 + n) return;
+    union H8 { chunk_t v; _Float16 e[8]; };
+    float mx = 0.f;
+    for (int kc = 0; kc < KT * 4; ++kc) {
+        H8 c;
+        c.v = tiles[chunk_index(r, kc, KT)];
+#pragma unroll
+        for (int j = 0; j < 8; ++j) mx = fmaxf(mx, fabsf((float)c.e[j]));
+    }
+    const float s = mx / 127.f;
+    const float inv = s > 0.f ? 1.f / s : 0.f;
+    double res2 = 0.0;
+    for (int kc8 = 0; kc8 < KT8 * 4; ++kc8) {
+        union { chunk_t v; int8_t e[16]; } out;
+#pragma unroll
+        for (int half = 0; half < 2; ++half) {
+            const int kc = kc8 * 2 + half;
+            H8 c;
+            c.v = kc < KT * 4 ? tiles[chunk_index(r, kc, KT)] : chunk_t{0u, 0u, 0u, 0u};
+#pragma unroll
+            for (int j = 0; j < 8; ++j) {
+                const float x = (float)c.e[j];
+                float qv = rintf(x * inv);
+                qv = fminf(fmaxf(qv, -127.f), 127.f);
+                out.e[half * 8 + j] = (int8_t)(int)qv;
+                const double d = (double)x - (double)s * (double)qv;
+                res2 += d * d;
+            }
+        }
+        tiles8[chunk_index(r, kc8, KT8)] = out.v;
+    }
+    const double n2 = norm2[r];
+    const double w = metric == HR_METRIC_COSINE ? (n2 > 0.0 ? 1.0 / sqrt(n2) : 0.0) : 1.0;
+    scale8[r] = (float)((double)s * w);
+    err8[r] = (float)(sqrt(res2) * w * (1.0 + 1e-6)) * 1.0000003f + 1e-37f;
+}
+
+__global__ void prep_queries_i8_kernel(const float* __restrict__ q, int B, int dim, int KT8, float m_prime,
+                                       chunk_t* __restrict__ qfrag8, float* __restrict__ q_sq, float* __restrict__ q_add) {
+    const int slot = blockIdx.x;
+    const int g = slot >> 4, col = slot & 15;
+    __shared__ float s_q[HR_MAX_DIM];
+    __shared__ float s_inv, s_scale;
+    __shared__ float s_red[256];
+    if (slot < B)
+        for (int k = threadIdx.x; k < dim; k += blockDim.x) s_q[k] = q[(int64_t)slot * dim + k];
+    __syncthreads();
+    if (threadIdx.x == 0) {
+        double s = 0.0;
+        if (slot < B)
+            for (int k = 0; k < dim; ++k) {
+                const double x = (double)s_q[k];
+                s = __dadd_rn(s, __dmul_rn(x, x));
+            }
+        s_inv = (s > 0.0) ? (float)(1.0 / sqrt(s)) : 0.0f;
+    }
+    __syncthreads();
+    const float inv = s_inv;
+    float mx = 0.f;
+    if (slot < B)
+        for (int k = threadIdx.x; k < dim; k += blockDim.x) {
+            s_q[k] = s_q[k] * inv;
+            mx = fmaxf(mx, fabsf(s_q[k]));
+        }
+    s_red[threadIdx.x] = mx;
+    __syncthreads();
+    if (threadIdx.x == 0) {
+        float m = 0.f;
+        for (int i = 0; i < (int)blockDim.x; ++i) m = fmaxf(m, s_red[i]);
+        s_scale = m / 127.f;
+    }
+    __syncthreads();
+    const float sq = s_scale;
+    const float isq = sq > 0.f ? 1.f / sq : 0.f;
+    double eta2 = 0.0;
+    for (int kc = threadIdx.x; kc < KT8 * 4; kc += blockDim.x) {
+        union { chunk_t v; int8_t e[16]; } hi, lo;
+#pragma unroll
+        for (int j = 0; j < 16; ++j) {
+            const int k = kc * 16 + j;
+            const float x = (slot < B && k < dim) ? s_q[k] : 0.f;
+            const float a = x * isq;
+            float hv = fminf(fmaxf(rintf(a), -127.f), 127.f);
+            float lv = fminf(fmaxf(rintf(254.f * (a - hv)), -127.f), 127.f);
+            hi.e[j] = (int8_t)(int)hv;
+            lo.e[j] = (int8_t)(int)lv;
+            const double eta = (double)x - (double)sq * ((double)hv + (double)lv / 254.0);
+            eta2 += eta * eta;
+        }
+        const int kt = kc >> 2, c = kc & 3;
+        chunk_t* dst = qfrag8 + (((int64_t)g * KT8 + kt) * 2) * kTileChunks + col + 16 * c;
+        dst[0] = hi.v;
+        dst[kTileChunks] = lo.v;
+    }
+    __shared__ double s_eta[256];
+    s_eta[threadIdx.x] = eta2;
+    __syncthreads();
+    if (threadIdx.x == 0) {
+        double e = 0.0;
+        for (int i = 0; i < (int)blockDim.x; ++i) e += s_eta[i];
+        const double b = ((sqrt(e) * (1.0 + 1e-9) + 0x1p-22) * 1.001 + 2e-6) * (double)m_prime;
+        q_sq[slot] = slot < B ? sq : 0.f;
+        q_add[slot] = slot < B ? (float)b * 1.0000003f + 1e-37f : 0.f;
+    }
+}
+
+template <int GQ>
+__global__ __launch_bounds__(512) void dense_scan_bigq_i8_kernel(
+    const chunk_t* __restrict__ tiles8, const chunk_t* __restrict__ qfrag8, const float* __restrict__ scale8,
+    const float* __restrict__ err8, const uint8_t* __restrict__ rowmask, float* __restrict__ gmax, int nq, int KT8,
+    int64_t n_rows, int64_t n_super, const float* __restrict__ q_sq, const float* __restrict__ q_add, float err_gain) {
+    constexpr int RS = 2, BKT = 1, PF = 2 * BKT;
+    constexpr int kPairs = kRowBlocksPerSuper / RS;
+    constexpr int kFrags = GQ * BKT * 2;
+    constexpr int kStage = kFrags / 8;
+    static_assert(kFrags % 8 == 0, "8 waves share the staging");
+    static_assert(PF == 2 * BKT, "two query chunks per trip of the ring");
+    extern __shared__ chunk_t lds_q[];
+    const int n_chunks = KT8 / BKT;
+    const int lane = threadIdx.x & 63, wid = threadIdx.x >> 6;
+    const int64_t wave = __builtin_amdgcn_readfirstlane((int)(blockIdx.x * 8 + wid));
+    const int64_t total_waves = (int64_t)gridDim.x * 8;
+    const int64_t gmax_stride = n_super * kRowBlocksPerSuper;
+    const int quad = lane >> 4;
+    const float NEG_INF = -__builtin_inff();
+    __shared__ float s_sq[16 * GQ], s_qb[16 * GQ];
+    if (threadIdx.x < 16 * GQ) {
+        s_sq[threadIdx.x] = q_sq[threadIdx.x];
+        s_qb[threadIdx.x] = q_add[threadIdx.x];
+    }
+    __shared__ f32x4_t s_gm[8][16 * GQ];
+    const int64_t n_rounds = (n_super + total_waves - 1) / total_waves;
+
+    const int64_t safe_group = wave % n_super;
+    int64_t pf_group = wave;
+    int pf_pair = 0, pf_kt = 0;
+    chunk_t ring[PF][RS];
+    auto prefetch = [&](int slot) {
+        const int64_t grp = pf_group < n_super ? pf_group : safe_group;
+        const int64_t rb = grp * kRowBlocksPerSuper + pf_pair * RS;
+#pragma unroll
+        for (int s = 0; s < RS; ++s)
+            ring[slot][s] = __builtin_nontemporal_load(tiles8 + ((rb + s) * KT8 + pf_kt) * kTileChunks + lane);
+        const bool wrap_kt = (pf_kt + 1 == KT8);
+        pf_kt = wrap_kt ? 0 : pf_kt + 1;
+        const bool wrap_pair = wrap_kt && (pf_pair + 1 == kPairs);
+        pf_pair = wrap_kt ? (wrap_pair ? 0 : pf_pair + 1) : pf_pair;
+        pf_group = wrap_pair ? pf_group + total_waves : pf_group;
+    };
+    auto q_src = [&](int chunk, int f) {
+        const int g = f / (2 * BKT), kk = (f >> 1) % BKT;
+        return qfrag8 + (((int64_t)g * KT8 + chunk * BKT + kk) * 2 + (f & 1)) * kTileChunks + lane;
+    };
+#pragma unroll
+    for (int i = 0; i < kStage; ++i) {
+        const int f = wid * kStage + i;
+        lds_q[f * kTileChunks + lane] = *q_src(0, f);
+    }
+#pragma unroll
+    for (int j = 0; j < PF; ++j) prefetch(j);
+    __syncthreads();
+    int cur = 0;
+
+    for (int64_t round = 0; round < n_rounds; ++round) {
+        const int64_t group = round * total_waves + wave;
+        const bool live = group < n_super;
+        const bool tail = live && ((group + 1) * kSuperRows > n_rows || rowmask != nullptr);
+#pragma unroll 1
+        for (int pair = 0; pair < kPairs; ++pair) {
+            i32x4_t acc[RS][GQ][2];
+#pragma unroll
+            for (int s = 0; s < RS; ++s)
+#pragma unroll
+                for (int g = 0; g < GQ; ++g) acc[s][g][0] = acc[s][g][1] = (i32x4_t){0, 0, 0, 0};
+            auto chunk_body = [&](auto SB, int kc) {
+                const int kn = (kc + 1 == n_chunks) ? 0 : kc + 1;
+                chunk_t stage[kStage];
+#pragma unroll
+                for (int i = 0; i < kStage; ++i) stage[i] = *q_src(kn, wid * kStage + i);
+                const chunk_t* qbuf = lds_q + cur * kFrags * kTileChunks;
+#pragma unroll
+                for (int j = 0; j < BKT; ++j) {
+                    chunk_t bn0 = qbuf[((0 * BKT + j) * 2 + 0) * kTileChunks + lane];
+                    chunk_t bn1 = qbuf[((0 * BKT + j) * 2 + 1) * kTileChunks + lane];
+#pragma unroll
+                    for (int f = 0; f < 2 * GQ; ++f) {
+                        union { chunk_t v; i32x4_t i; } b;
+                        b.v = bn0;
+                        bn0 = bn1;
+                        if (f + 2 < 2 * GQ) bn1 = qbuf[((((f + 2) >> 1) * BKT + j) * 2 + (f & 1)) * kTileChunks + lane];
+#pragma unroll
+                        for (int s = 0; s < RS; ++s) {
+                            union { chunk_t v; i32x4_t i; } a;
+                            a.v = ring[decltype(SB)::value + j][s];
+                            acc[s][f >> 1][f & 1] = __builtin_amdgcn_mfma_i32_16x16x64_i8(a.i, b.i, acc[s][f >> 1][f & 1], 0, 0, 0);
+                        }
+                        __builtin_amdgcn_sched_barrier(0);
+                    }
+                    prefetch(decltype(SB)::value + j);
+                }
+                chunk_t* qn = lds_q + (cur ^ 1) * kFrags * kTileChunks;
+#pragma unroll
+                for (int i = 0; i < kStage; ++i) qn[(wid * kStage + i) * kTileChunks + lane] = stage[i];
+                __syncthreads();
+                cur ^= 1;
+            };
+#pragma unroll 1
+            for (int kc = 0; kc < n_chunks; kc += 2) {
+                chunk_body(std::integral_constant<int, 0>{}, kc);
+                chunk_body(std::integral_constant<int, BKT>{}, kc + 1);
+            }
+            if (live) {
+#pragma unroll
+                for (int s = 0; s < RS; ++s) {
+                    const int64_t rblock = group * kRowBlocksPerSuper + pair * RS + s;
+                    const int64_t row0 = rblock * kRowsPerBlock + quad * 4;
+                    const f32x4_t sc = *reinterpret_cast<const f32x4_t*>(scale8 + row0);
+                    const f32x4_t er = *reinterpret_cast<const f32x4_t*>(err8 + row0);
+                    float ok[4] = {1.f, 1.f, 1.f, 1.f};
+                    if (tail) {
+#pragma unroll
+                        for (int r = 0; r < 4; ++r) {
+                            int64_t row = row0 + r;
+                            bool v = row < n_rows;
+                            if (v && rowmask) v = (rowmask[row >> 3] >> (row & 7)) & 1;
+                            ok[r] = v ? 1.f : 0.f;
+                        }
+                    }
+#pragma unroll
+                    for (int g = 0; g < GQ; ++g) {
+                        const float sq = s_sq[16 * g + (lane & 15)], qb = s_qb[16 * g + (lane & 15)];
+                        float mr = NEG_INF;
+#pragma unroll
+                        for (int r = 0; r < 4; ++r) {
+                            const float dot = (float)acc[s][g][0][r] + (float)acc[s][g][1][r] * (1.f / 254.f);
+                            float v = dot * (sq * sc[r]) + (er[r] * err_gain + qb);
+                            v = (ok[r] != 0.f) ? v : NEG_INF;
+                            mr = fmaxf(mr, v);
+                        }
+                        mr = col4_max(mr);
+                        if (lane < 16) reinterpret_cast<float*>(&s_gm[wid][16 * g + lane])[pair * RS + s] = mr;
+                    }
+                }
+            }
+        }
+        if (live) {
+#pragma unroll
+            for (int hq = 0; hq < (16 * GQ) / 64; ++hq) {
+                const int q = hq * 64 + lane;
+                const f32x4_t v = s_gm[wid][q];
+                if (q < nq) *reinterpret_cast<f32x4_t*>(gmax + (int64_t)q * gmax_stride + group * kRowBlocksPerSuper) = v;
+            }
+        }
+    }
+}
+
+}
diff --git a/advanced-rag-milvus_amd/csrc/finish.h b/advanced-rag-milvus_amd/csrc/finish.h
--- a/advanced-rag-milvus_amd/csrc/finish.h
+++ b/advanced-rag-milvus_amd/csrc/finish.h
@@ -10,6 +10,8 @@
 constexpr int kFinishMaxSlots = 4096;
 constexpr int kFinishMaxCand = 256;
 constexpr int kFinishMaxBuckets = 12288;
+constexpr int kBoundMaxCand = 1024;
+constexpr int kBoundExtraKeys = 2048;
 
 struct FinishMod {
     int kind;
@@ -31,6 +33,7 @@
     const float* q_val;
     int q_cap;
     int64_t n_rows;
+    unsigned* bound_stats;
 };
 struct FinishPair {
     FinishMod m[2];
@@ -49,7 +52,7 @@
                              (finish_sparse_hashed(m.q_cap) ? (size_t)sparse_hash_slots(m.q_cap) * 8 : (size_t)m.q_cap * 8);
             region_b = region_b > s ? region_b : s;
         } else {
-            const size_t s = (size_t)m.dim * 4;
+            const size_t s = (size_t)m.dim * 4 + (m.kind == 2 && m.sel.two_level ? (size_t)m.sel.n_buckets * 4 : 0);
             region_b = region_b > s ? region_b : s;
         }
     }
@@ -94,6 +97,10 @@
     __shared__ int32_t sel_bucket[HR_MAX_TOPK * 2];
     __shared__ uint64_t sel[HR_MAX_TOPK];
     __shared__ int32_t s_cand[kFinishMaxCand];
+    __shared__ int32_t s_cand2[kBoundMaxCand];
+    __shared__ int s_n2, s_nkeys, s_over;
+    __shared__ unsigned long long s_thr_key;
+    __shared__ float s_thr;
     const FinishMod& a = p.m[blockIdx.y];
     const int q = blockIdx.x, tid = threadIdx.x;
     const int n_slots = a.sel.C * a.group_rows;
@@ -116,7 +123,86 @@
     }
 #endif
 
-    if (a.kind == 0) {
+    if (a.kind == 2) {
+        float* qq = s_bmax + (a.sel.two_level ? a.sel.n_buckets : 0);
+        for (int k = tid; k < a.dim; k += kFinishThreads) qq[k] = a.q[(int64_t)q * a.dim + k];
+        if (tid == 0) s_n2 = 0, s_nkeys = 0, s_over = 0;
+        __syncthreads();
+        const double qn2 = a.qn2[q];
+        for (int slot = tid; slot < n_live_slots; slot += kFinishThreads) {
+            float sc = 0.f;
+            int32_t row = -1;
+            const bool ok = refine_dense_slot<_Float16>(a.tiles, a.KT, a.dim, qq, qn2, a.norm2, a.rowmask, s_cand, a.group_rows,
+                                                        a.n_rows, a.metric, slot, &sc, &row);
+            s_key[slot] = ok ? rank_key(sc, (uint32_t)row) : 0ull;
+        }
+        __syncthreads();
+        const int K = a.topk.K;
+        const uint64_t kth = K <= n_slots ? block_kth_largest([&](int64_t i) -> uint64_t { return s_key[i]; }, n_slots, K, sh) : 0ull;
+        if (tid == 0) {
+            float thr = -__builtin_inff();
+            if (kth != 0ull) {
+                double sk = (double)key_score(kth);
+                if (a.topk.norm_mode == 1) sk = qn2 > 0.0 ? sk / sqrt(qn2) : 0.0;
+                const double b = sk - 2.0 * (double)a.topk.eps_abs - 4e-7 * fabs(sk) - 1e-30;
+                thr = (float)b;
+                if ((double)thr > b) thr = unord_f32(ord_f32(thr) - 1u);
+            }
+            s_thr = thr;
+            s_thr_key = kth;
+        }
+        __syncthreads();
+        const float thr = s_thr;
+        const uint64_t thr_key = s_thr_key;
+        {
+            const int lane = tid & 63, wid = __builtin_amdgcn_readfirstlane(tid >> 6);
+            constexpr int NW = kFinishThreads / 64;
+            const float* gm = a.sel.gmax + (int64_t)q * a.sel.n_groups;
+            const int C1 = a.sel.C;
+            for (int64_t b = wid; b < a.sel.n_buckets; b += NW) {
+                if (a.sel.two_level && !(s_bmax[b] >= thr)) continue;
+                const int64_t g = b * kBucketGroups + lane;
+                bool take = g < a.sel.n_groups && gm[g] >= thr;
+                if (take)
+                    for (int j = 0; j < C1; ++j) take = take && s_cand[j] != (int32_t)g;
+                if (take) {
+                    const int pos = atomicAdd(&s_n2, 1);
+                    if (pos < kBoundMaxCand) s_cand2[pos] = (int32_t)g;
+                    else s_over = 1;
+                }
+            }
+        }
+        __syncthreads();
+        const int n2 = min(s_n2, kBoundMaxCand);
+        const int extra = p.key_slots - n_slots;
+        for (int slot = tid; slot < n2 * a.group_rows; slot += kFinishThreads) {
+            float sc = 0.f;
+            int32_t row = -1;
+            const bool ok = refine_dense_slot<_Float16>(a.tiles, a.KT, a.dim, qq, qn2, a.norm2, a.rowmask, s_cand2, a.group_rows,
+                                                        a.n_rows, a.metric, slot, &sc, &row);
+            const uint64_t kk = ok ? rank_key(sc, (uint32_t)row) : 0ull;
+            if (kk > thr_key) {
+                const int pos = atomicAdd(&s_nkeys, 1);
+                if (pos < extra) s_key[n_slots + pos] = kk;
+                else s_over = 1;
+            }
+        }
+        __syncthreads();
+        if (tid == 0) {
+            a.sel.a_cut[q] = s_over ? __builtin_inff() : thr;
+            if (a.bound_stats) {
+                atomicAdd(&a.bound_stats[0], (unsigned)n2);
+                atomicMax(&a.bound_stats[1], (unsigned)s_n2);
+                if (s_over) atomicAdd(&a.bound_stats[2], 1u);
+                atomicAdd(&a.bound_stats[3], 1u);
+            }
+        }
+        __syncthreads();
+        TopkArgs t = a.topk;
+        t.n = n_slots + min(s_nkeys, extra);
+        select_topk_block(t, q, [&](int64_t i) -> uint64_t { return s_key[i]; }, sh, sel);
+        return;
+    } else if (a.kind == 0) {
         float* qq = s_bmax;
         for (int k = tid; k < a.dim; k += kFinishThreads) qq[k] = a.q[(int64_t)q * a.dim + k];
         __syncthreads();
diff --git a/advanced-rag-milvus_amd/csrc/hbmrag.hip b/advanced-rag-milvus_amd/csrc/hbmrag.hip
--- a/advanced-rag-milvus_amd/csrc/hbmrag.hip
+++ b/advanced-rag-milvus_amd/csrc/hbmrag.hip
@@ -3,6 +3,7 @@
 #include <hip/hip_runtime.h>
 
 #include <algorithm>
+#include <atomic>
 #include <chrono>
 #include <cmath>
 #include <cstdarg>
@@ -27,6 +28,7 @@
 #include "encoder_layer.h"
 #include "scan_plan.h"
 #include "dense.h"
+#include "dense_i8.h"
 #include "encoder_ops.h"
 #include "filter.h"
 #include "finish.h"
@@ -109,6 +111,7 @@
     struct Workspace* sparse_ws = nullptr;
     DevBuf qfrag, qn2, gmax, bmax, cand, acut, cscore, crow, flags, qscale, qeps, qfloor, pq_n, pq_idx, pq_w;
     DevBuf qcoef, dqeps;
+    DevBuf qfrag8, q_sq, q_add;
     DevBuf rbounds, rhi, rlo;
     DevBuf d_radius, d_rfilter;
     DevBuf d_q, d_ids, d_scores, d_mask;
@@ -135,6 +138,10 @@
     DevBuf tiles, scale, norm2, max_norm;
     int64_t cap_rows = 0, n_rows = 0, n_normed = 0;
     float max_row_norm = 0.f;
+    DevBuf tiles8, scale8, err8, bound_stats;
+    int KT8 = 0;
+    int64_t cap8_rows = 0, n_q8 = 0;
+    mutable std::atomic<int> widest_scan_B{0}, widest_scan_i8{0};
     DevBuf stage;
     DevBuf bad_row;
     hipStream_t ingest_stream = nullptr;
@@ -462,6 +469,8 @@
 int g_no_trim = 0;
 int g_group_rows = 0;
 int g_no_range_clamp = 0;
+int g_finish_mode = 0;
+int g_i8 = 0;
 
 inline int64_t bucket_count(int64_t n_groups) { return (n_groups + kBucketGroups - 1) / kBucketGroups; }
 int launch_group_select_pair(hr_index* h, hipStream_t s, int B, const GroupSelPair& p) {
@@ -526,6 +535,7 @@
     int GR;
     int64_t n_groups;
     int C;
+    bool bound;
     const uint8_t* mask;
     TopkArgs topk;
     const float* d_q;
@@ -564,14 +574,23 @@
     return HR_OK;
 }
 inline int64_t dense_super_groups(const hr_index* h) { return (h->n_rows + kSuperRows - 1) / kSuperRows; }
+bool dense_narrow_pass(const hr_index* h, int B, int k, int C, bool ranged) {
+    return g_i8 && !ranged && h->KT8 > 0 && h->n_rows > 0 && h->n_q8 == h->n_rows && B > 64 && B <= 128 &&
+           C == candidate_groups_for_k(k) && g_finish_mode != 1 && g_dense_kernels == 0 && h->group_rows_override == 0 &&
+           bucket_count(dense_super_groups(h) * kRowBlocksPerSuper) <= kFinishMaxBuckets;
+}
 int dense_side(hr_index* h, Workspace* ws, const float* d_q, int B, int k, int C, const uint8_t* d_mask, const OutLists& out,
                FinishSide* f, bool ranged = false) {
-    const int GR = group_rows_for(h, h->n_rows);
+    const bool bound = dense_narrow_pass(h, B, k, C, ranged);
+    const int GR = bound ? kRowsPerBlock : group_rows_for(h, h->n_rows);
+    if (bound) C = std::min(C, kFinishMaxCand);
     HR_TRY(side_common(h, ws, B, k, C, GR, dense_super_groups(h) * (kSuperRows / GR), d_mask, out, f));
+    f->bound = bound;
     f->d_q = d_q;
     f->ph_select = PH_GSEL, f->ph_refine = PH_REFINE, f->ph_topk = PH_TOPK;
     TopkArgs& t = f->topk;
     dense_eps(h, &t.eps_abs, &t.norm_mode);
+    if (bound) t.eps_abs = 1e-6f * (h->metric == HR_METRIC_COSINE ? 1.f : h->max_row_norm * 1.0001f);
     t.cut_floor = -INFINITY;
     t.eps_abs_q = t.norm_mode == 2 ? ws->dqeps.as<float>() : nullptr;
     t.qn2 = ws->qn2.as<double>();
@@ -608,7 +627,7 @@
     a.two_level = f.n_groups > f.C && a.n_buckets > f.C;
     a.cand = f.ws->cand.as<int32_t>();
     a.a_cut = f.ws->acut.as<float>();
-    a.K_trim = g_no_trim ? 0 : f.topk.K;
+    a.K_trim = (g_no_trim || f.bound) ? 0 : f.topk.K;
     a.eps_abs = f.topk.eps_abs;
     a.eps_rel = f.topk.eps_rel;
     a.eps_abs_q = f.topk.eps_abs_q;
@@ -616,7 +635,8 @@
 }
 FinishMod finish_mod(const hr_index* h, const FinishSide& f) {
     FinishMod m{};
-    m.kind = f.sparse;
+    m.kind = f.sparse ? 1 : f.bound ? 2 : 0;
+    m.bound_stats = f.bound ? h->bound_stats.as<unsigned>() : nullptr;
     m.group_rows = f.GR;
     m.sel = sel_args(f);
     m.topk = f.topk;
@@ -677,19 +697,20 @@
 
 enum { PHASE_SCAN = 1, PHASE_FINISH = 2, PHASE_PREP = 4, PHASE_ALL = 7 };
 
-int g_finish_mode = 0;
 bool finish_fused_ok(int B, int n_mod, const FinishSide& f) {
     if (g_finish_mode == 1) return false;
+    if (f.bound) return true;
     return ((int64_t)B * n_mod >= 64 || g_finish_mode == 2) && f.C <= kFinishMaxCand && (int64_t)f.C * f.GR <= kFinishMaxSlots &&
            bucket_count(f.n_groups) <= kFinishMaxBuckets;
 }
 int launch_finish(hr_index* h, hipStream_t s, int B, FinishPair& p) {
     p.key_slots = 0;
-    for (int i = 0; i < p.n; ++i) p.key_slots = std::max(p.key_slots, p.m[i].sel.C * p.m[i].group_rows);
+    for (int i = 0; i < p.n; ++i)
+        p.key_slots = std::max(p.key_slots, p.m[i].sel.C * p.m[i].group_rows + (p.m[i].kind == 2 ? kBoundExtraKeys : 0));
     const size_t lds = finish_lds_bytes(p);
     static bool attr_set = false;
     if (!attr_set) {
-        HIP_TRY(h, hipFuncSetAttribute((const void*)finish_kernel, hipFuncAttributeMaxDynamicSharedMemorySize, 96 * 1024));
+        HIP_TRY(h, hipFuncSetAttribute((const void*)finish_kernel, hipFuncAttributeMaxDynamicSharedMemorySize, 128 * 1024));
         attr_set = true;
     }
     hipLaunchKernelGGL(finish_kernel, dim3(B, p.n), dim3(kFinishThreads), lds, s, p);
@@ -707,6 +728,17 @@
         for (int i = 0; i < n; ++i) p.m[i] = finish_mod(h, f[i]);
         return launch_finish(h, s, B, p);
     }
+    if (n == 2 && (f[0].bound || f[1].bound)) {
+        const int b = f[0].bound ? 0 : 1;
+        {
+            Span sp(h, s, PH_FINISH);
+            FinishPair p{};
+            p.n = 1;
+            p.m[0] = finish_mod(h, f[b]);
+            HR_TRY(launch_finish(h, s, B, p));
+        }
+        return finish_enqueue(h, s, B, &f[1 - b], 1);
+    }
     {
         Span sp(h, s, f[0].ph_select);
         GroupSelPair p{};
@@ -726,6 +758,13 @@
         HR_TRY(launch_topk_pair(h, s, B, p));
     }
     return HR_OK;
+}
+
+inline void note_scan(const hr_index* h, int nq, int i8) {
+    if (nq >= h->widest_scan_B.load(std::memory_order_relaxed)) {
+        h->widest_scan_B.store(nq, std::memory_order_relaxed);
+        h->widest_scan_i8.store(i8, std::memory_order_relaxed);
+    }
 }
 
 int dense_search_enqueue(hr_index* h, Workspace* ws, hipStream_t s, const float* d_q, int B, int k,
@@ -779,6 +818,39 @@
                            d_qeps, rt_eps, rp);
         HIP_TRY(h, hipGetLastError());
     }
+    if (f.bound) {
+        constexpr int GQ = 8;
+        HIP_TRY(h, ws->qfrag8.ensure((size_t)GQ * h->KT8 * 2 * kTileChunks * sizeof(chunk_t)));
+        HIP_TRY(h, ws->q_sq.ensure((size_t)16 * GQ * sizeof(float)));
+        HIP_TRY(h, ws->q_add.ensure((size_t)16 * GQ * sizeof(float)));
+        if (phases & PHASE_PREP) {
+            Span sp(h, s, PH_PREP);
+            const float m_prime = h->metric == HR_METRIC_COSINE ? 1.f : h->max_row_norm * 1.0001f;
+            hipLaunchKernelGGL(prep_queries_i8_kernel, dim3(16 * GQ), dim3(256), 0, s, d_q, B, (int)h->dim, h->KT8, m_prime,
+                               ws->qfrag8.as<chunk_t>(), ws->q_sq.as<float>(), ws->q_add.as<float>());
+            HIP_TRY(h, hipGetLastError());
+        }
+        if (phases & PHASE_SCAN) {
+            Span sp(h, s, PH_SCAN);
+            auto kern = dense_scan_bigq_i8_kernel<GQ>;
+            const size_t lds = (size_t)2 * GQ * 2 * 1024;
+            static bool attr_set = false;
+            if (!attr_set) {
+                HIP_TRY(h, hipFuncSetAttribute((const void*)kern, hipFuncAttributeMaxDynamicSharedMemorySize, (int)lds));
+                attr_set = true;
+            }
+            const int64_t n_super = dense_super_groups(h);
+            const int64_t blocks = std::max<int64_t>(1, std::min<int64_t>((n_super + 7) / 8, (int64_t)scan_cus(h)));
+            hipLaunchKernelGGL(kern, dim3((unsigned)blocks), dim3(512), lds, s, h->tiles8.as<chunk_t>(), ws->qfrag8.as<chunk_t>(),
+                               h->scale8.as<float>(), h->err8.as<float>(), d_mask, ws->gmax.as<float>(), B, h->KT8, h->n_rows,
+                               n_super, ws->q_sq.as<float>(), ws->q_add.as<float>(), i8_err_gain(h->KT8));
+            HIP_TRY(h, hipGetLastError());
+            note_scan(h, B, 1);
+        }
+        if (scan_done) HIP_TRY(h, hipEventRecord(scan_done, s));
+        return (phases & PHASE_FINISH) ? finish_enqueue(h, s, B, &f, 1) : HR_OK;
+    }
+    if (phases & PHASE_SCAN) note_scan(h, std::min(B, chunk_q), 0);
     for (int c0 = 0; (phases & PHASE_SCAN) && c0 < B; c0 += chunk_q) {
         const int nq = std::min(chunk_q, B - c0);
         Span sp(h, s, PH_SCAN);
@@ -937,6 +1009,36 @@
     h->scale = std::move(scale);
     h->norm2 = std::move(norm2);
     h->cap_rows = rows;
+    return HR_OK;
+}
+
+int build_narrow_copy(hr_index* h) {
+    if (h->KT8 == 0 || !g_i8 || h->n_q8 >= h->n_normed) return HR_OK;
+    hipStream_t s = h->ingest_stream;
+    if (h->cap8_rows != h->cap_rows) {
+        DevBuf t8, s8, e8;
+        const size_t tb = (size_t)(h->cap_rows / kRowsPerBlock) * h->KT8 * 1024;
+        if (t8.alloc_exact(tb) != hipSuccess || s8.alloc_exact((size_t)h->cap_rows * 4) != hipSuccess ||
+            e8.alloc_exact((size_t)h->cap_rows * 4) != hipSuccess) {
+            (void)hipGetLastError();
+            return fail(h, HR_ENOMEM, "cannot allocate the narrow scan copy for %lld rows (%zu bytes)", (long long)h->cap_rows, tb);
+        }
+        HIP_TRY(h, hipMemsetAsync(t8.p, 0, t8.cap, s));
+        HIP_TRY(h, hipMemsetAsync(s8.p, 0, s8.cap, s));
+        HIP_TRY(h, hipMemsetAsync(e8.p, 0, e8.cap, s));
+        h->tiles8 = std::move(t8);
+        h->scale8 = std::move(s8);
+        h->err8 = std::move(e8);
+        h->cap8_rows = h->cap_rows;
+        h->n_q8 = 0;
+    }
+    const int64_t n = h->n_normed - h->n_q8;
+    hipLaunchKernelGGL(quantize_rows_kernel, dim3((unsigned)((n + 255) / 256)), dim3(256), 0, s, h->tiles.as<chunk_t>(), h->KT,
+                       h->KT8, (int)h->dim, h->n_q8, n, h->metric, h->norm2.as<double>(), h->tiles8.as<chunk_t>(),
+                       h->scale8.as<float>(), h->err8.as<float>());
+    HIP_TRY(h, hipGetLastError());
+    HIP_TRY(h, hipStreamSynchronize(s));
+    h->n_q8 = h->n_normed;
     return HR_OK;
 }
 
@@ -1262,6 +1364,7 @@
         const int tile_elems = 4 * elems_per_chunk(dtype);
         h->KT = (int)round_up((dim + tile_elems - 1) / tile_elems, 4);
     }
+    if (dim > 0 && dtype == HR_F16 && metric != HR_METRIC_L2 && dim % 64 == 0) h->KT8 = i8_tiles_per_row(dim);
     h->group_rows_override = g_group_rows;
     DeviceGuard dg(device);
     hipDeviceProp_t prop;
@@ -1271,6 +1374,7 @@
     if (hipStreamCreateWithFlags(&h->ingest_stream, hipStreamNonBlocking) != hipSuccess ||
         h->max_norm.alloc_exact(4) != hipSuccess || hipMemset(h->max_norm.p, 0, 4) != hipSuccess ||
         h->bad_row.alloc_exact(8) != hipSuccess || hipMemset(h->bad_row.p, 0xFF, 8) != hipSuccess ||
+        h->bound_stats.alloc_exact(16) != hipSuccess || hipMemset(h->bound_stats.p, 0, 16) != hipSuccess ||
         h->idle_post.alloc_exact(sizeof idle) != hipSuccess ||
         hipMemcpy(h->idle_post.p, idle, sizeof idle, hipMemcpyHostToDevice) != hipSuccess) {
         int rc = fail(nullptr, HR_EHIP, "device %d initialisation failed: %s", device, hipGetErrorString(hipGetLastError()));
@@ -1355,7 +1459,8 @@
     std::unique_lock<std::shared_mutex> lk(h->rw);
     DeviceGuard dg(h->device);
     hipStream_t s = h->ingest_stream;
-    if ((h->dim > 0 && h->n_normed < h->n_rows) || (h->sparse_dim > 0 && h->n_sparse_built != h->n_sparse))
+    if ((h->dim > 0 && (h->n_normed < h->n_rows || (h->KT8 > 0 && h->n_q8 < h->n_rows))) ||
+        (h->sparse_dim > 0 && h->n_sparse_built != h->n_sparse))
         HIP_TRY(h, hipDeviceSynchronize());
     if (h->dim > 0 && h->n_normed < h->n_rows) {
         const int64_t n = h->n_rows - h->n_normed;
@@ -1372,6 +1477,9 @@
         std::memcpy(&h->max_row_norm, &bits, 4);
         h->n_normed = h->n_rows;
     }
+    HR_TRY(build_narrow_copy(h));
+    h->widest_scan_B.store(0, std::memory_order_relaxed);
+    h->widest_scan_i8.store(0, std::memory_order_relaxed);
     if (h->sparse_dim > 0 && (h->n_sparse_built != h->n_sparse || h->n_csr != h->n_sparse)) HR_TRY(build_sparse(h));
     h->finalized = true;
     return HR_OK;
@@ -1438,6 +1546,7 @@
     h->compact_ms[0] = h->compact_ms[2] = 0.f;
     if (timed) (void)hipEventElapsedTime(&h->compact_ms[0], ev.e[0], ev.e[1]);
 
+    int narrow_rc = HR_OK;
     if (dense && kd < h->n_rows) {
         h->tiles = std::move(nd.tiles);
         h->scale = std::move(nd.scale);
@@ -1446,6 +1555,11 @@
         h->cap_rows = nd.cap_rows;
         h->n_rows = h->n_normed = kd;
         std::memcpy(&h->max_row_norm, &norm_bits, 4);
+        h->tiles8.release();
+        h->scale8.release();
+        h->err8.release();
+        h->cap8_rows = h->n_q8 = 0;
+        narrow_rc = build_narrow_copy(h);
     }
     if (kept_dense) *kept_dense = h->n_rows;
     if (sparse && ks < h->n_sparse) {
@@ -1472,7 +1586,7 @@
         h->finalized = true;
     }
     h->compact_ms[1] = wall_ms(t_call);
-    return HR_OK;
+    return narrow_rc;
 }
 
 namespace {
@@ -1671,13 +1785,25 @@
 int64_t hr_device_bytes(const hr_index* h) {
     if (!h) return 0;
     size_t t = 0;
-    for (const DevBuf* b : {&h->tiles, &h->scale, &h->norm2, &h->s_indptr, &h->s_idx, &h->s_val, &h->rt_off,
-                            &h->range_base, &h->post})
+    for (const DevBuf* b : {&h->tiles, &h->scale, &h->norm2, &h->tiles8, &h->scale8, &h->err8, &h->s_indptr, &h->s_idx,
+                            &h->s_val, &h->rt_off, &h->range_base, &h->post})
         t += b->cap;
     return (int64_t)t;
 }
+int hr_bound_finish_stats(hr_index* h, uint64_t out[4]) {
+    if (!h || !out) return fail(h, HR_EINVAL, "null argument");
+    DeviceGuard dg(h->device);
+    unsigned v[4] = {0u, 0u, 0u, 0u};
+    HIP_TRY(h, hipDeviceSynchronize());
+    HIP_TRY(h, hipMemcpy(v, h->bound_stats.p, sizeof v, hipMemcpyDeviceToHost));
+    HIP_TRY(h, hipMemset(h->bound_stats.p, 0, sizeof v));
+    out[0] = v[3], out[1] = v[0], out[2] = v[1], out[3] = v[2];
+    return HR_OK;
+}
 int64_t hr_dense_scan_bytes(const hr_index* h) {
     if (!h || h->dim == 0) return 0;
+    if (h->widest_scan_i8.load(std::memory_order_relaxed))
+        return h->n_rows * (int64_t)h->KT8 * 64 + h->n_rows * 8;
     const int64_t dpad = (int64_t)h->KT * 4 * elems_per_chunk(h->dtype);
     return h->n_rows * dpad * (int64_t)elem_size(h->dtype) + h->n_rows * 4;
 }
@@ -2235,6 +2361,9 @@
         case HR_DEBUG_NO_RANGE_CLAMP:
             g_no_range_clamp = value != 0;
             return HR_OK;
+        case HR_DEBUG_I8_SCAN:
+            g_i8 = value != 0;
+            return HR_OK;
         case HR_DEBUG_FAIL_NEXT_BUILD:
             if (!h) return fail(nullptr, HR_EINVAL, "null handle");
             h->fault_inject = value ? 1 : 0;
diff --git a/include/hbmrag.h b/include/hbmrag.h
--- a/include/hbmrag.h
+++ b/include/hbmrag.h
@@ -308,7 +308,7 @@
 HR_API int hr_set_scan_cus(hr_index* h, int n_cus);
 
 enum { HR_DEBUG_FINISH_MODE = 1, HR_DEBUG_FAIL_NEXT_BUILD = 2, HR_DEBUG_DENSE_KERNELS = 3, HR_DEBUG_SPARSE_RPB = 4,
-       HR_DEBUG_GROUP_ROWS = 5, HR_DEBUG_NO_TRIM = 6, HR_DEBUG_NO_RANGE_CLAMP = 7 };
+       HR_DEBUG_GROUP_ROWS = 5, HR_DEBUG_NO_TRIM = 6, HR_DEBUG_NO_RANGE_CLAMP = 7, HR_DEBUG_I8_SCAN = 8 };
 HR_API int hr_debug_option(hr_index* h, int key, int value);
 
 #define HR_N_PHASES 10
@@ -316,6 +316,7 @@
 HR_API int hr_last_kernel_ms(hr_index* h, float* out_ms, int n);
 HR_API int hr_last_compact_ms(hr_index* h, float* out_ms, int n);
 HR_API int64_t hr_dense_scan_bytes(const hr_index* h);
+HR_API int hr_bound_finish_stats(hr_index* h, uint64_t out[4]);
 
 #ifdef __cplusplus
 }
```

After: 33670. 0.989x the previous value.
